# wangxuanx/Face-Diffusion-Model

Measured on AMD Instinct MI355X. Metric: animated frames/sec (1000-step DDPM, VOCASET FDM) at 1/2/4/8 MI355X, higher is better.
Workload: dtype bf16; 1 GPU; cfg2: vocaset FDM, 4 clips/GPU x 200 latent frames, 1000-step DDPM, random-init weights, synthetic audio-encoder features, Philox noise; global_batch=4, latent_frames=200, diffusion_steps=1000, parallelism=clip-shard x1

## Files before the change

face-diffusion-model_amd/csrc/fdm_hip.hip:

```cpp
#include <hip/hip_runtime.h>

#include <cstdarg>
#include <cstdio>
#include <functional>

#include "elementwise.hpp"
#include "window.hpp"
#include "slots.hpp"
#include "host.hpp"

namespace fdm {
thread_local std::string g_err;
int fail(int code, const char* fmt, ...) {
  char buf[512];
  va_list ap;
  va_start(ap, fmt);
  vsnprintf(buf, sizeof(buf), fmt, ap);
  va_end(ap);
  g_err = buf;
  return code;
}
}

namespace {
// ... 10 lines not shown
struct fdm_prog {
  std::vector<Op> ops;
  hipGraph_t graph = nullptr;
  hipGraphExec_t exec = nullptr;
};

namespace {

thread_local fdm_prog* g_rec = nullptr;

int submit(Op op, void* stream, const char* what) {
  if (g_rec) {
    g_rec->ops.push_back(std::move(op));
    return FDM_OK;
  }
  hipError_t e = op((hipStream_t)stream);
  if (e != hipSuccess) return hip_fail(e, what);
  return FDM_OK;
}

bool aligned16(const void* p) { return (((uintptr_t)p) & 15) == 0; }

}

extern "C" {

const char* fdm_last_error(void) { return g_err.c_str(); }
int fdm_version(void) { return 105; }

int fdm_abi_struct_size(const char* name) {
  if (!name) return fdm::fail(FDM_ERR_ARG, "abi_struct_size: null name");
  const std::string n(name);
  if (n == "fdm_sched_args") return (int)sizeof(fdm_sched_args);
  if (n == "fdm_gemm_args") return (int)sizeof(fdm_gemm_args);
  if (n == "fdm_attn_args") return (int)sizeof(fdm_attn_args);
  if (n == "fdm_ln_args") return (int)sizeof(fdm_ln_args);
  if (n == "fdm_model_desc") return (int)sizeof(fdm_model_desc);
  if (n == "fdm_sample_args") return (int)sizeof(fdm_sample_args);
  if (n == "fdm_vq_desc") return (int)sizeof(fdm_vq_desc);
  if (n == "fdm_slot_group_args") return (int)sizeof(fdm_slot_group_args);
  if (n == "fdm_slot_bank_args") return (int)sizeof(fdm_slot_bank_args);
  return fdm::fail(FDM_ERR_ARG, "abi_struct_size: unknown struct '%s'", name);
}

int fdm_device_ok(void) {
  int n = 0;
  if (hipGetDeviceCount(&n) != hipSuccess || n <= 0) return 0;
  hipDeviceProp_t prop;
  if (hipGetDeviceProperties(&prop, 0) != hipSuccess) return 0;
  return strncmp(prop.gcnArchName, "gfx950", 6) == 0 ? 1 : 0;
}

static bool gemm_act_heavy_host(int act) { return act == FDM_ACT_MISH || act == FDM_ACT_GELU_ERF || act == FDM_ACT_GELU_TANH; }

int fdm_op_gemm(const fdm_gemm_args* a, void* stream) {
  if (!a || !a->A || !a->W) return fail(FDM_ERR_ARG, "gemm: null operand");
  if (a->M <= 0 || a->N <= 0 || a->K <= 0) return fail(FDM_ERR_SHAPE, "gemm: M,N,K must be positive (%d,%d,%d)", a->M, a->N, a->K);
  if (!kind_ok(a->dtype)) return fail(FDM_ERR_ARG, "gemm: bad dtype %d", a->dtype);
  const bool split = kind(a->dtype).planes == 2;
  const int bk = kind(a->dtype).bk, epc = kind(a->dtype).epc;
  if (split && (a->a_lo_off <= 0 || a->w_lo_off <= 0 || a->a_lo_off % epc || a->w_lo_off % epc))
    return fail(FDM_ERR_ARG, "gemm: split operands need positive a_lo_off / w_lo_off (multiples of 8 elements)");
  if (split && a->out_t && a->out_t_lo_off <= 0) return fail(FDM_ERR_ARG, "gemm: split out_t needs out_t_lo_off");
  if (a->K % bk) return fail(FDM_ERR_SHAPE, "gemm: K=%d not a multiple of %d", a->K, bk);
  if (a->lda % epc || a->ldw % epc || !aligned16(a->A) || !aligned16(a->W)) return fail(FDM_ERR_ARG, "gemm: operands need 16-byte aligned rows");
  if (a->lda < 0 || a->ldw < 0 || a->lda > 0x7fffffffLL || a->ldw > 0x7fffffffLL) return fail(FDM_ERR_SHAPE, "gemm: lda / ldw are passed to the kernel as 32-bit element counts");
  if (a->a_batch_stride % epc || a->w_batch_stride % epc) return fail(FDM_ERR_ARG, "gemm: batch strides need 16-byte alignment");
  if (!a->out_f32 && !a->out_t && !a->out_vp && !a->out_kp) return fail(FDM_ERR_ARG, "gemm: no output");
  if (a->out_kp || a->out_vp) {
    const int hi = a->out_vp ? a->vp_col0 : a->N;
    if (a->kv_hd <= 0 || a->kv_hd % 16 || a->kv_L <= 0 || a->kv_Lpad < a->kv_L || a->kv_Lpad % 32 || a->M % a->kv_L)
      return fail(FDM_ERR_SHAPE, "gemm: bad packed K/V geometry (hd %d, L %d, Lpad %d)", a->kv_hd, a->kv_L, a->kv_Lpad);
    if (a->out_vp && (a->vp_col0 < 0 || a->vp_col0 % 4 || (a->N - a->vp_col0) % a->kv_hd)) return fail(FDM_ERR_SHAPE, "gemm: bad packed V column range");
    if (a->out_kp && (a->kp_col0 < 0 || a->kp_col0 % 4 || hi < a->kp_col0 || (hi - a->kp_col0) % a->kv_hd)) return fail(FDM_ERR_SHAPE, "gemm: bad packed K column range");
    if (!aligned16(a->out_kp) || !aligned16(a->out_vp)) return fail(FDM_ERR_ARG, "gemm: packed K/V buffers must be 16-byte aligned");
    if (a->dtype == FDM_F16X3 && (a->kv_lo_off <= 0 || a->kv_lo_off % 8)) return fail(FDM_ERR_ARG, "gemm: split packed K/V outputs need kv_lo_off");
  }
  if (a->bias && !aligned16(a->bias)) return fail(FDM_ERR_ARG, "gemm: bias must be 16-byte aligned");
  if (a->ln_stat_in && (a->ln_nparts <= 0 || a->ln_dim <= 0)) return fail(FDM_ERR_ARG, "gemm: ln_stat_in needs ln_nparts and ln_dim");
  if ((a->ln_colsum || a->rln_gamma) && !a->ln_stat_in) return fail(FDM_ERR_ARG, "gemm: LayerNorm folding needs ln_stat_in");
  if (a->rln_gamma && (!a->rln_beta || !a->resid)) return fail(FDM_ERR_ARG, "gemm: rln_gamma needs rln_beta and resid");
  if ((a->stat_out || a->ln_stat_in) && (a->batch > 1 || a->out_batch_stride)) return fail(FDM_ERR_ARG, "gemm: LayerNorm folding is not batched");
  if (a->tile < 0 || (a->tile & FDM_TILE_ID_MASK) > FDM_TILE_MAX) return fail(FDM_ERR_ARG, "gemm: unknown tile %d", a->tile);
  if (a->sched_fuse) {
    const fdm_sched_args& sc = a->sched;
    if (sc.mode != 0 && sc.mode != 1 && sc.mode != 3) return fail(FDM_ERR_ARG, "gemm: fused scheduler supports mode 0 (DDPM), 1 (DDIM) and 3 (table-driven)");
    if (!a->resid || !a->out_f32 || a->N % 64 || a->ldo_f32 != a->N || a->ldr != a->N || a->resid_row_mod || a->batch > 1 ||
        !aligned16(a->resid) || !aligned16(a->out_f32) || (a->out_t && (a->ldo_t != a->N || !aligned16(a->out_t))))
      return fail(FDM_ERR_SHAPE, "gemm: fused scheduler needs resid = x_t and out_f32 = x_{t-1} as dense [M, N] arrays, N %% 64 == 0");
    if (gemm_act_heavy_host(a->act) || a->stat_out || a->out_kp || a->out_vp || a->rln_gamma)
      return fail(FDM_ERR_ARG, "gemm: fused scheduler cannot be combined with Mish/GELU, stat_out, packed K/V or rln outputs");
    if (sc.mode == 0 && (!sc.c1 || !sc.c2 || !sc.sigma)) return fail(FDM_ERR_ARG, "gemm: fused DDPM needs c1, c2, sigma");
    if (sc.mode == 1 && (!sc.sra || !sc.srm1 || !sc.sqrt_an || !sc.c_n)) return fail(FDM_ERR_ARG, "gemm: fused DDIM needs sra, srm1, sqrt_an, c_n");
    if (sc.mode == 0 && !sc.noise && sc.n_per_clip <= 0) return fail(FDM_ERR_ARG, "gemm: fused DDPM with Philox noise needs n_per_clip");
    if (sc.mode == 3 && (!sc.lm_a || !sc.lm_b || !sc.lm_c || !sc.lm_s || !sc.x0_hist || !aligned16(sc.x0_hist)))
      return fail(FDM_ERR_ARG, "gemm: fused table-driven sampler needs lm_a, lm_b, lm_c, lm_s and a 16-byte aligned x0_hist [M, N]");
    if (sc.mode == 3 && !sc.noise && sc.n_per_clip <= 0) return fail(FDM_ERR_ARG, "gemm: fused table-driven sampler with Philox noise needs n_per_clip");
  }
  if (a->ksplit < 0 || a->ksplit > 4) return fail(FDM_ERR_ARG, "gemm: ksplit %d outside 0..4", a->ksplit);
  if (a->ksplit > 1) {
    const int tl = a->tile & FDM_TILE_ID_MASK;
    if (a->batch > 1 || a->out_batch_stride || a->act != FDM_ACT_NONE || !a->out_f32 || a->out_t || a->out_kp || a->out_vp || a->stat_out || a->ln_stat_in ||
        a->sched_fuse || a->resid_row_mod || (a->tile & FDM_TILE_GENERAL))
      return fail(FDM_ERR_ARG, "gemm: ksplit needs a plain launch (one batch, no activation, out_f32 as the only output, no folds)");
    if ((a->K / bk) % a->ksplit) return fail(FDM_ERR_SHAPE, "gemm: ksplit %d does not divide the %d k-tiles of K=%d", a->ksplit, a->K / bk, a->K);
    if (a->N % 64 || a->ldo_f32 % 4 || !aligned16(a->out_f32) || a->ksplit_stride % 4 || a->ksplit_stride < (long long)(a->M - 1) * a->ldo_f32 + a->N ||
        (a->resid && (a->ldr % 4 || !aligned16(a->resid))))
      return fail(FDM_ERR_SHAPE, "gemm: ksplit needs N %% 64 == 0, 16-byte aligned rows and ksplit_stride >= one output plane");
    if (tl != 0 && tl != FDM_TILE_64x64 && tl != FDM_TILE_64x64_S2 && tl != FDM_TILE_32x64_S3)
      return fail(FDM_ERR_ARG, "gemm: ksplit runs on the 64-column tiles (FDM_TILE_64x64, FDM_TILE_64x64_S2, FDM_TILE_32x64_S3), not tile %d", tl);
  }
  if (a->batch2 < 0) return fail(FDM_ERR_ARG, "gemm: negative batch2");
  if (a->batch2 >= 1) {
    const int tl = a->tile & FDM_TILE_ID_MASK;
    if (a->ksplit > 1 || a->out_kp || a->out_vp || a->stat_out || a->ln_stat_in || a->sched_fuse || a->resid_row_mod || a->incr_counter)
      return fail(FDM_ERR_ARG, "gemm: batch2 cannot be combined with ksplit, packed K/V, LayerNorm folds, the fused scheduler or resid_row_mod");
    if (a->a_batch_stride2 % epc) return fail(FDM_ERR_ARG, "gemm: a_batch_stride2 needs 16-byte alignment");
    if (tl != 0 && tl != FDM_TILE_64x64 && tl != FDM_TILE_64x64_S2 && tl != FDM_TILE_128x64)
      return fail(FDM_ERR_ARG, "gemm: batch2 runs on the 64-column tiles (FDM_TILE_64x64, FDM_TILE_64x64_S2, FDM_TILE_128x64), not tile %d", tl);
    if (a->batch < 1) return fail(FDM_ERR_ARG, "gemm: batch2 needs batch >= 1 (the group count of the second batch level)");
  }
  fdm_gemm_args c = *a;
  return submit([c](hipStream_t s) { return fdm::gemm_launch(c, s); }, stream, "gemm");
}

int fdm_gemm_heuristic_tile(const fdm_gemm_args* a) {
  if (!a) return fail(FDM_ERR_ARG, "gemm_heuristic_tile: null argument");
  return fdm::gemm_heuristic_tile_of(*a);
}

int fdm_op_attention(const fdm_attn_args* a, void* stream) {
  if (!a || !a->Q || !a->Kp || !a->Vp || !a->O) return fail(FDM_ERR_ARG, "attention: null operand");
  if (a->hd != 64 && a->hd != 128 && a->hd != 256) return fail(FDM_ERR_SHAPE, "attention: head_dim %d unsupported (64, 128, 256)", a->hd);
  if (a->B <= 0 || a->H <= 0 || a->L <= 0) return fail(FDM_ERR_SHAPE, "attention: B,H,L must be positive");
  if (a->Lpad < a->L || a->Lpad % 32) return fail(FDM_ERR_SHAPE, "attention: Lpad=%d must be a multiple of 32 >= L", a->Lpad);
  if (!kind_ok(a->dtype)) return fail(FDM_ERR_ARG, "attention: bad dtype %d (FDM_F32, FDM_BF16, FDM_F16X3, FDM_F16)", a->dtype);
  if (a->o_split && (a->dtype != FDM_F32 || a->o_split != FDM_F16X3 || a->o_lo_off <= 0))
    return fail(FDM_ERR_ARG, "attention: o_split needs dtype FDM_F32, a split kind and o_lo_off");
  if (a->dtype == FDM_F16X3 && (a->q_lo_off <= 0 || a->kv_lo_off <= 0 || a->o_lo_off <= 0 || a->q_lo_off % 8 || a->kv_lo_off % 8 || a->o_lo_off % 4))
    return fail(FDM_ERR_ARG, "attention: split operands need q_lo_off, kv_lo_off and o_lo_off");
  if (a->q_lo_off > 0x7fffffffLL || a->kv_lo_off > 0x7fffffffLL || a->ldq > 0x7fffffffLL)
    return fail(FDM_ERR_SHAPE, "attention: q_lo_off, kv_lo_off and ldq are passed to the kernel as 32-bit element counts");
  const int epc = kind(a->dtype).epc;
  if (a->ldq % epc || a->ldo % 4 || !aligned16(a->Q) || !aligned16(a->Kp) || !aligned16(a->Vp) || !aligned16(a->O))
    return fail(FDM_ERR_ARG, "attention: operands need 16-byte aligned rows");
  if (a->slopes && a->period <= 0) return fail(FDM_ERR_ARG, "attention: period must be positive");
  if (a->lens && (a->causal || (a->hd != 64 && a->hd != 128)))
    return fail(FDM_ERR_ARG, "attention: per-clip lengths need causal = 0 and head_dim 64 or 128");
  fdm_attn_args c = *a;
  return submit([c](hipStream_t s) { return fdm::attn_launch(c, s); }, stream, "attention");
}

int fdm_op_pack_kv(const void* K, long long ldk, const void* V, long long ldv, void* Kp, void* Vp,
                   int B, int H, int L, int Lpad, int hd, int dtype, void* stream) {
  if (!K || !V || !Kp || !Vp) return fail(FDM_ERR_ARG, "pack_kv: null operand");
  if (B <= 0 || H <= 0 || L <= 0 || Lpad < L || Lpad % 32 || hd <= 0 || hd % 16) return fail(FDM_ERR_SHAPE, "pack_kv: bad geometry");
  if (dtype != FDM_F32 && dtype != FDM_BF16) return fail(FDM_ERR_ARG, "pack_kv: bad dtype %d", dtype);
  return submit([=](hipStream_t s) {
    return dtype == FDM_BF16 ? fdm::pack_kv_launch_bf16(K, ldk, V, ldv, Kp, Vp, B, H, L, Lpad, hd, s)
                             : fdm::pack_kv_launch_f32(K, ldk, V, ldv, Kp, Vp, B, H, L, Lpad, hd, s);
  }, stream, "pack_kv");
}

int fdm_op_layernorm(const fdm_ln_args* a, void* stream) {
  if (!a || !a->x || !a->gamma || !a->beta) return fail(FDM_ERR_ARG, "layernorm: null operand");
  if (a->d != 256 && a->d != 512 && a->d != 768 && a->d != 1024) return fail(FDM_ERR_SHAPE, "layernorm: d=%d unsupported (256, 512, 768, 1024)", a->d);
  if (a->M <= 0) return fail(FDM_ERR_SHAPE, "layernorm: M must be positive");
  if (!a->y_f32 && !a->y_t) return fail(FDM_ERR_ARG, "layernorm: no output");
  if (!kind_ok(a->dtype)) return fail(FDM_ERR_ARG, "layernorm: bad dtype %d", a->dtype);
  if (a->y_t && a->dtype == FDM_F16X3 && (a->y_t_lo_off <= 0 || a->y_t_lo_off % 4)) return fail(FDM_ERR_ARG, "layernorm: split y_t needs y_t_lo_off");
  if (a->add_mat_group < 0 || a->add_mat_wrap < 0 ||
      (a->add_mat_group > 0 && (a->add_mat_L <= 0 || a->add_mat_group % a->add_mat_L || (a->add_mat_wrap > 0 && a->add_mat_wrap % a->add_mat_group))))
    return fail(FDM_ERR_SHAPE, "layernorm: shared add_mat needs add_mat_L | add_mat_group | add_mat_wrap (got %d, %d, %d)", a->add_mat_L, a->add_mat_group, a->add_mat_wrap);
  if (a->x_planes < 0 || a->x_planes > 4 || (a->x_planes > 1 && (a->x_plane_stride < (long long)a->M * a->d || a->x_plane_stride % 4)))
    return fail(FDM_ERR_ARG, "layernorm: x_planes %d (0..4) needs x_plane_stride >= M * d, a multiple of 4", a->x_planes);
  if (a->clip_step && (a->clip_rows <= 0 || a->clip_step_stride <= 0 || a->clip_wrap < 0 || (a->clip_wrap > 0 && a->clip_wrap % a->clip_rows)))
    return fail(FDM_ERR_SHAPE, "layernorm: clip_step needs clip_rows > 0, clip_step_stride > 0 and clip_rows | clip_wrap (got %d, %d, %d)", a->clip_rows, a->clip_step_stride, a->clip_wrap);
  if (a->clip_step && a->act != FDM_ACT_NONE && a->act != FDM_ACT_RELU) return fail(FDM_ERR_ARG, "layernorm: clip_step runs with FDM_ACT_NONE / FDM_ACT_RELU only");
  fdm_ln_args c = *a;
  return submit([c](hipStream_t s) {
    switch (c.dtype) {
      case FDM_BF16: return fdm::ln_launch_t<fdm::bf16>(c, s);
      case FDM_F16X3: return fdm::ln_launch_t<fdm::f16x3_t>(c, s);
      case FDM_F16: return fdm::ln_launch_t<fdm::f16>(c, s);
      default: return fdm::ln_launch_t<float>(c, s);
    }
  }, stream, "layernorm");
}

int fdm_op_sched_step(const fdm_sched_args* a, void* stream) {
  if (!a || !a->x0 || !a->x_out) return fail(FDM_ERR_ARG, "sched: null operand");
  if (a->n <= 0 || a->n % 4) return fail(FDM_ERR_SHAPE, "sched: n=%lld must be a positive multiple of 4", a->n);
  if (a->mode == 0 && (!a->x || !a->c1 || !a->c2 || !a->sigma)) return fail(FDM_ERR_ARG, "sched: DDPM tables missing");
  if (a->mode == 1 && (!a->x || !a->sra || !a->srm1 || !a->sqrt_an || !a->c_n)) return fail(FDM_ERR_ARG, "sched: DDIM tables missing");
  if (a->mode == 3 && (!a->x || !a->lm_a || !a->lm_b || !a->lm_c || !a->lm_s || !a->x0_hist)) return fail(FDM_ERR_ARG, "sched: table-driven sampler needs lm_a, lm_b, lm_c, lm_s, x0_hist");
  if (a->mode < 0 || a->mode > 3) return fail(FDM_ERR_ARG, "sched: bad mode %d", a->mode);
  if (a->mode == 3 && !a->noise && (a->n_per_clip <= 0 || a->n_per_clip % 4)) return fail(FDM_ERR_SHAPE, "sched: n_per_clip must be a positive multiple of 4");
  if (a->mode == 0 && !a->noise && (a->n_per_clip <= 0 || a->n_per_clip % 4)) return fail(FDM_ERR_SHAPE, "sched: n_per_clip must be a positive multiple of 4");
  if (a->x_out_t && !kind_ok(a->out_dtype)) return fail(FDM_ERR_ARG, "sched: bad out_dtype %d", a->out_dtype);
  if (a->x_out_t && a->out_dtype == FDM_F16X3 && (a->x_out_t_lo_off <= 0 || a->x_out_t_lo_off % 4)) return fail(FDM_ERR_ARG, "sched: split x_out_t needs x_out_t_lo_off");
  fdm_sched_args c = *a;
  return submit([c](hipStream_t s) { return fdm::sched_launch(c, s); }, stream, "sched");
}

int fdm_op_slot_sched(const fdm_sched_args* a, const int* state, const unsigned long long* keys, int n_slots, void* stream) {
  if (!a || !a->x0 || !a->x || !a->x_out || !state || !keys) return fail(FDM_ERR_ARG, "slot_sched: null operand");
  if (a->noise) return fail(FDM_ERR_ARG, "slot_sched: injected noise is not supported (Philox keyed per slot)");
  if (a->mode != 0 && a->mode != 1 && a->mode != 3) return fail(FDM_ERR_ARG, "slot_sched: mode %d (0 DDPM, 1 DDIM, 3 table-driven)", a->mode);
  if (n_slots < 1 || a->n_per_clip <= 0 || a->n_per_clip % 4 || a->n != (long long)n_slots * a->n_per_clip)
    return fail(FDM_ERR_SHAPE, "slot_sched: n=%lld must be n_slots=%d x n_per_clip=%lld (a multiple of 4)", a->n, n_slots, a->n_per_clip);
  if (a->mode == 0 && (!a->c1 || !a->c2 || !a->sigma)) return fail(FDM_ERR_ARG, "slot_sched: DDPM tables missing");
// ... 531 lines not shown
```

face-diffusion-model_amd/csrc/gemm.hpp:

```cpp
#pragma once
#include <cstdlib>
#include <cstring>

#include "common.hpp"
#include "sched.hpp"
#include "../../include/fdm_hip.h"

namespace fdm {

template <int BM, int BN> constexpr int gemm_ln_scratch_bytes() { return BM * 2 * 4; }
template <typename T, int BM, int BN> constexpr int gemm_epi_ring_bytes() {
  using KK = typename Opnd<T>::KV;
  return BM * BN * (int)sizeof(typename Opnd<KK>::E) * Opnd<KK>::NP + BM * 2 * (BN / 16) * 4;
}

template <int BM>
__device__ __forceinline__ void gemm_load_rowstats(const fdm_gemm_args& p, int m0, float* rowstat) {
  if (!p.ln_stat_in) return;
  const int t = threadIdx.x;
  if (t < BM) {
    const int m = min(m0 + t, p.M - 1);
    float s = 0.f, q = 0.f;
    typedef __attribute__((ext_vector_type(2))) float f32x2;
    for (int i0 = 0; i0 < p.ln_nparts; i0 += 16) {
      f32x2 v[16];
#pragma unroll
      for (int i = 0; i < 16; ++i) {
        const int ii = min(i0 + i, p.ln_nparts - 1);
        v[i] = *(const f32x2*)(p.ln_stat_in + ((size_t)ii * p.M + m) * 2);
      }
#pragma unroll
      for (int i = 0; i < 16; ++i)
        if (i0 + i < p.ln_nparts) { s += v[i][0]; q += v[i][1]; }
    }
    const float inv = 1.f / (float)p.ln_dim;
    const float mu = s * inv;
    const float var = fmaxf(q * inv - mu * mu, 0.f);
    rowstat[2 * t] = mu;
    rowstat[2 * t + 1] = 1.f / sqrtf(var + p.ln_eps);
  }
  asm volatile("s_waitcnt lgkmcnt(0)" ::: "memory");
}

template <int MI, int NI> struct EpiPre { f32x4 csv[NI], bv[NI], gmv[NI], btv[NI], rv[MI][NI]; SchedCoef sc; };

template <typename T, int BM, int BN, int WM, int WN, int SCHED = 0>
__device__ __forceinline__ void gemm_epi_preload(const fdm_gemm_args& p, int m0, int n0, int z, int wm, int wn, int g, int r16,
                                                 bool ln_capable, EpiPre<BM / WM / 16, BN / WN / 16>& e) {
  constexpr int MI = BM / WM / 16, NI = BN / WN / 16;
  if constexpr (SCHED != 0) e.sc = sched_coef_load<SCHED == 2>(p.sched);
  const int M = p.M, N = p.N;
  const bool use_ln = ln_capable && p.ln_stat_in;
  const float* bias = p.bias ? p.bias + (size_t)z * p.bias_batch_stride : nullptr;
  const size_t ocol = (size_t)z * p.out_batch_stride;
  const bool vec_r = p.resid && (p.ldr % 4 == 0) && (((uintptr_t)(p.resid + ocol)) % 16 == 0);
  const bool pre_cs = use_ln && p.ln_colsum, pre_rln = use_ln && p.rln_gamma && p.resid;
#pragma unroll
  for (int ni = 0; ni < NI; ++ni) {
    const int n = n0 + wn * (BN / WN) + ni * 16 + 4 * g;
    const bool full = (n + 3 < N);
    const f32x4 zero = f32x4{0.f, 0.f, 0.f, 0.f};
    e.csv[ni] = (pre_cs && full) ? *(const f32x4*)(p.ln_colsum + n) : zero;
    e.bv[ni] = (bias && full) ? *(const f32x4*)(bias + n) : zero;
    e.gmv[ni] = (pre_rln && full) ? *(const f32x4*)(p.rln_gamma + n) : zero;
    e.btv[ni] = (pre_rln && full) ? *(const f32x4*)(p.rln_beta + n) : zero;
#pragma unroll
    for (int mi = 0; mi < MI; ++mi) {
      const int m = m0 + wm * (BM / WM) + mi * 16 + r16;
      const size_t rrow = p.resid_row_mod > 0 ? (size_t)(min(m, M - 1) % p.resid_row_mod) : (size_t)min(m, M - 1);
      e.rv[mi][ni] = (p.resid && vec_r && full && m < M) ? *(const f32x4*)(p.resid + ocol + rrow * p.ldr + n) : zero;
    }
  }
}

template <bool HEAVY, typename T> __device__ __forceinline__ float gemm_act(float v, int act) {
  if constexpr (!HEAVY) {
    return act == ACT_RELU ? fmaxf(v, 0.f) : (act == ACT_LEAKY02 ? (v > 0.f ? v : 0.2f * v) : v);
  } else if constexpr (is_fast16<T>::value) {
    if (act == ACT_MISH) {
      const float sp = v > 20.f ? v : __logf(1.f + __expf(v));
      return v * (1.f - 2.f / (1.f + __expf(2.f * sp)));
    }
    if (act == ACT_GELU_TANH) {
      const float c = 0.7978845608028654f * (v + 0.044715f * v * v * v);
      return v * (0.5f * (2.f - 2.f / (1.f + __expf(2.f * c))));
    }
    return act_apply_t<T>(v, act);
  } else {
    return act_apply(v, act);
  }
}
__host__ __device__ inline bool gemm_act_is_heavy(int act) { return act == ACT_MISH || act == ACT_GELU_ERF || act == ACT_GELU_TANH; }

constexpr int GEMM_LEAN = 1, GEMM_KV = 2, GEMM_FOLD = 4, GEMM_KSPLIT = 8, GEMM_B2 = 16, GEMM_LM = 32;
template <int MODE> struct KSliceArgs;
template <> struct KSliceArgs<0> {
  const fdm_gemm_args& a;
  __device__ __forceinline__ KSliceArgs(const fdm_gemm_args& p, int, int) : a(p) {}
};
template <> struct KSliceArgs<1> {
  fdm_gemm_args a;
  __device__ __forceinline__ KSliceArgs(const fdm_gemm_args& p, int slice, int) : a(p) {
    a.out_f32 = p.out_f32 + (size_t)slice * p.ksplit_stride;
    if (slice > 0) { a.bias = nullptr; a.resid = nullptr; }
  }
};
template <> struct KSliceArgs<2> {
  fdm_gemm_args a;
  __device__ __forceinline__ KSliceArgs(const fdm_gemm_args& p, int c, int out_t_elem_bytes) : a(p) {
    const size_t off = (size_t)c * p.out_batch_stride2;
    if (p.out_f32) a.out_f32 = p.out_f32 + off;
    if (p.resid) a.resid = p.resid + off;
    if (p.out_t) a.out_t = (char*)p.out_t + off * out_t_elem_bytes;
  }
};
template <typename T, int BM, int BN, int WM = 2, int WN = 2, bool HEAVY = true, bool SCHED = false, int SPEC = 0>
__device__ __forceinline__ void gemm_epilogue(const fdm_gemm_args& p, f32x4 (&acc)[BM / WM / 16][BN / WN / 16],
                                              const EpiPre<BM / WM / 16, BN / WN / 16>& e, int m0, int n0, int z,
                                              int wm, int wn, int g, int r16, float* rowstat = nullptr, char* tile_lds = nullptr) {
  constexpr int MI = BM / WM / 16, NI = BN / WN / 16;
  constexpr bool LEAN = (SPEC & GEMM_LEAN) != 0;
  constexpr bool KVC = !LEAN || (SPEC & GEMM_KV), FOLDC = !LEAN || (SPEC & GEMM_FOLD);
  using E = typename Opnd<T>::E;
  using KK = typename Opnd<T>::KV;
  using KV = typename Opnd<KK>::E;
  constexpr int KNP = Opnd<KK>::NP;
  const int M = p.M, N = p.N;
  constexpr int EPC_T = 16 / (int)sizeof(KV);
  const bool vt_tile = KVC && tile_lds && p.out_vp && n0 >= p.vp_col0 && n0 + BN <= N && (p.kv_L % EPC_T == 0);
  KV* tl = (KV*)tile_lds;
  float* comb = tile_lds ? (float*)(tile_lds + BM * BN * (int)sizeof(KV) * KNP) : nullptr;
  const bool use_ln = FOLDC && rowstat && p.ln_stat_in;
  const bool do_stat = FOLDC && rowstat && comb && p.stat_out;
  if (vt_tile || do_stat) __syncthreads();
  const float* bias = p.bias ? p.bias + (size_t)z * p.bias_batch_stride : nullptr;
  const size_t ocol = (size_t)z * p.out_batch_stride;
  const bool vec_f32 = p.out_f32 && (p.ldo_f32 % 4 == 0) && (((uintptr_t)(p.out_f32 + ocol)) % 16 == 0);
  const bool vec_t = p.out_t && (p.ldo_t % 4 == 0) && (((uintptr_t)((E*)p.out_t + ocol)) % (4 * sizeof(E)) == 0) &&
                     (Opnd<T>::NP == 1 || p.out_t_lo_off % 4 == 0);
  const bool vec_r = p.resid && (p.ldr % 4 == 0) && (((uintptr_t)(p.resid + ocol)) % 16 == 0);
  const int kv_H = p.out_vp ? (N - p.vp_col0) / p.kv_hd : 0;
  const size_t kv_blk = (size_t)p.kv_Lpad * p.kv_hd;
  const int kcol_lo = p.out_kp ? p.kp_col0 : N, kcol_hi = p.out_kp ? (p.out_vp ? p.vp_col0 : N) : N;
  const bool pre_cs = use_ln && p.ln_colsum, pre_rln = use_ln && p.rln_gamma && p.resid;
  const f32x4 (&csv)[NI] = e.csv; const f32x4 (&bv)[NI] = e.bv; const f32x4 (&gmv)[NI] = e.gmv; const f32x4 (&btv)[NI] = e.btv;
  const f32x4 (&rv)[MI][NI] = e.rv;
  const int kv_mode = (!KVC || (!p.out_kp && !p.out_vp)) ? 0
                    : (n0 + BN <= (p.out_kp ? kcol_lo : p.vp_col0)) ? 0
                    : (p.out_kp && n0 >= kcol_lo && n0 + BN <= kcol_hi) ? 1
                    : vt_tile ? 2
                    : (p.out_vp && n0 >= p.vp_col0 && n0 + BN <= N) ? 3 : -1;
  const bool lean = LEAN || (kv_mode >= 0 && n0 + BN <= N && (vec_f32 || !p.out_f32) && (vec_t || !p.out_t) && (vec_r || !p.resid) &&
                            (p.kv_hd % 16 == 0 || kv_mode != 1));
  if (lean) {
    const int ncol = n0 + wn * (BN / WN) + 4 * g;
    const int KH = (kv_mode == 1) ? (kcol_hi - kcol_lo) / p.kv_hd : 1;
#pragma unroll
    for (int mi = 0; mi < MI; ++mi) {
      const int lrow = wm * (BM / WM) + mi * 16 + r16;
      const int m = m0 + lrow;
      if (m >= M) continue;
      const float mu = use_ln ? rowstat[2 * lrow] : 0.f, rs = use_ln ? rowstat[2 * lrow + 1] : 1.f;
      float* o32 = p.out_f32 ? p.out_f32 + ocol + (size_t)m * p.ldo_f32 + ncol : nullptr;
      E* ot = p.out_t ? (E*)p.out_t + ocol + (size_t)m * p.ldo_t + ncol : nullptr;
      KV* okp = nullptr;
      int kv_l = 0;
      if (kv_mode == 1) {
        const int kv_b = m / p.kv_L;
        kv_l = m - kv_b * p.kv_L;
        okp = (KV*)p.out_kp + (size_t)kv_b * KH * kv_blk;
      } else if (kv_mode == 3) {
        const int kv_b = m / p.kv_L;
        kv_l = m - kv_b * p.kv_L;
        okp = (KV*)p.out_vp + (size_t)kv_b * kv_H * kv_blk;
      }
#pragma unroll
      for (int ni = 0; ni < NI; ++ni) {
        f32x4 v = acc[mi][ni];
        if (pre_cs) v = (v - mu * csv[ni]) * rs;
        if (bias) v += bv[ni];
        if (p.act != ACT_NONE) {
#pragma unroll
          for (int j = 0; j < 4; ++j) v[j] = gemm_act<HEAVY, T>(v[j], p.act);
        }
        if constexpr (SCHED) {
          v = sched_update4<(SPEC & GEMM_LM) != 0>(p.sched, e.sc, v, rv[mi][ni], (long long)m * N + (ncol + ni * 16));
        } else {
          if (p.resid) v += pre_rln ? (rv[mi][ni] - mu) * rs * gmv[ni] + btv[ni] : rv[mi][ni];
        }
        if (do_stat) {
          const float fs = rows_sum((v[0] + v[1]) + (v[2] + v[3]));
          const float fq = rows_sum((v[0] * v[0] + v[1] * v[1]) + (v[2] * v[2] + v[3] * v[3]));
          if (g == 0) { float* cb = comb + ((size_t)(wn * NI + ni) * BM + lrow) * 2; cb[0] = fs; cb[1] = fq; }
        }
        if (kv_mode == 2) {
          const int nl = wn * (BN / WN) + ni * 16 + 4 * g;
#pragma unroll
          for (int j = 0; j < 4; ++j) store_opnd1<KK>(tl + (nl + j) * BM + lrow, BM * BN, v[j]);
          continue;
        }
        if (kv_mode == 1) {
          const int cc = ncol + ni * 16 - kcol_lo;
          const int h = cc / p.kv_hd, e2 = cc - h * p.kv_hd;
          store_opnd4<KK>(okp + (size_t)h * kv_blk + kp_offset<KV>(kv_l, e2, p.kv_hd), p.kv_lo_off, v);
          continue;
        }
        if (kv_mode == 3) {
          const int cc = ncol + ni * 16 - p.vp_col0;
          const int h = cc / p.kv_hd, e2 = cc - h * p.kv_hd;
#pragma unroll
// ... 81 lines not shown
          if (n + j >= N) break;
          const int cc = n + j - p.vp_col0;
          const int h = cc / p.kv_hd, e = cc - h * p.kv_hd;
          store_opnd1<KK>((KV*)p.out_vp + (size_t)(kv_b * kv_H + h) * kv_blk + vp_offset<KV>(kv_l, e, p.kv_hd), p.kv_lo_off, v[j]);
        }
        continue;
      }
      if (p.out_f32) {
        float* op = p.out_f32 + ocol + (size_t)m * p.ldo_f32 + n;
        if (full && vec_f32) {
          *(f32x4*)op = v;
        } else {
          for (int j = 0; j < 4; ++j)
            if (n + j < N) op[j] = v[j];
        }
      }
      if (p.out_t) {
        E* op = (E*)p.out_t + ocol + (size_t)m * p.ldo_t + n;
        if (full && vec_t) {
          store_opnd4<T>(op, p.out_t_lo_off, v);
        } else {
          for (int j = 0; j < 4; ++j)
            if (n + j < N) store_opnd1<T>(op + j, p.out_t_lo_off, v[j]);
        }
      }
    }
  }
  }
  if (vt_tile) {
    __syncthreads();
    constexpr int CPR = BM / EPC_T;
    for (int c = threadIdx.x; c < BN * CPR; c += WM * WN * 64) {
      const int nl = c / CPR, ml = (c % CPR) * EPC_T;
      const int m = m0 + ml;
      if (m >= M) continue;
      const int b = m / p.kv_L, l = m - b * p.kv_L;
      const int cc = n0 + nl - p.vp_col0;
      const int h = cc / p.kv_hd, e = cc - h * p.kv_hd;
#pragma unroll
      for (int pl = 0; pl < KNP; ++pl)
        *(u32x4*)((KV*)p.out_vp + (size_t)pl * p.kv_lo_off + (size_t)(b * kv_H + h) * kv_blk + vp_offset<KV>(l, e, p.kv_hd)) =
            *(const u32x4*)(tl + pl * BM * BN + nl * BM + ml);
    }
  }
  if (do_stat) {
    __syncthreads();
    const int t = threadIdx.x;
    if (t < BM && m0 + t < M) {
#pragma unroll
      for (int gq = 0; gq < BN / 64; ++gq) {
        if (n0 + gq * 64 >= N) break;
        float s = 0.f, q = 0.f;
#pragma unroll
        for (int f = 0; f < 4; ++f) { s += comb[((size_t)(gq * 4 + f) * BM + t) * 2]; q += comb[((size_t)(gq * 4 + f) * BM + t) * 2 + 1]; }
        float* so = p.stat_out + ((size_t)(n0 / 64 + gq) * M + (m0 + t)) * 2;
        so[0] = s; so[1] = q;
      }
    }
  }
}

#ifndef FDM_LW_VARIANT
#define FDM_LW_VARIANT 0
#endif
typedef __attribute__((address_space(1))) const void* gptr_t;
typedef __attribute__((address_space(3))) void* lptr_t;

template <int N> __device__ __forceinline__ void wait_vmcnt() { asm volatile("s_waitcnt vmcnt(%0)" ::"n"(N) : "memory"); }

template <typename T, int BM, int BN, int WM, int WN, int NST, int KCH = 8, bool HEAVY = false, bool SCHED = false, int SPEC = 0, int LW = 0>
__global__ __launch_bounds__(64 * (WM * WN + LW)) void gemm_glds_kernel(const void* pA, const void* pW, long long p_a_lo_off, long long p_w_lo_off,
                                                                        int pM, int pN, int pK, int p_lda, int p_ldw, const fdm_gemm_args p) {
  using E = typename Opnd<T>::E;
  constexpr int NP = Opnd<T>::NP;
  constexpr int NW = WM * WN;
  constexpr int ROWB = KCH * 16;
  constexpr int RPI = 1024 / ROWB;
  constexpr int MI = BM / WM / 16, NI = BN / WN / 16;
  constexpr int NA = BM / RPI, NWP = BN / RPI;
  constexpr int IW = LW > 0 ? LW : NW;
  constexpr bool UNEVEN = NA % IW != 0;
  static_assert(NWP % IW == 0 && BM % RPI == 0 && MI >= 1 && NI >= 1, "tile does not fit the wave grid");
  constexpr int A_IPW = (NA + IW - 1) / IW, W_IPW = NWP / IW;
  constexpr int P = NP * (A_IPW + W_IPW), P_LO = NP * (A_IPW - 1 + W_IPW);
  constexpr int STAGE = NP * (BM + BN) * ROWB;
  static_assert(NST * STAGE >= gemm_epi_ring_bytes<T, BM, BN>(), "epilogue staging does not fit in the ring");
  constexpr bool EARLY_READS = NP * (KCH / 4) * (MI + NI) <= 12;
  extern __shared__ __attribute__((aligned(16))) char smem[];
#ifdef FDM_GEMM_STAMPS
  const unsigned long long t_first = wall_clock64();
#endif
  float* rowstat = (float*)(smem + NST * STAGE);

  const int tid = threadIdx.x, lane = tid & 63;
#ifdef FDM_GEMM_STAMPS
  unsigned long long* stamps = (!p.incr_counter && p.incr_table) ? (unsigned long long*)p.incr_table + (size_t)(blockIdx.y * gridDim.x + blockIdx.x) * 8 : nullptr;
  if (stamps && tid == 0) { stamps[0] = wall_clock64(); stamps[5] = t_first; }
#endif
  const int wave_id = __builtin_amdgcn_readfirstlane(tid >> 6);
  const bool loader = LW > 0 && wave_id >= NW;
  const int wave = LW > 0 ? (loader ? wave_id - NW : 0) : wave_id;
  const int wm = wave_id / WN, wn = wave_id % WN;
  const int g = lane >> 4, r16 = lane & 15;
  constexpr bool KSP = (SPEC & GEMM_KSPLIT) != 0, B2 = (SPEC & GEMM_B2) != 0;
  int z = KSP ? 0 : blockIdx.z;
  int by = blockIdx.y, bx = blockIdx.x, c2 = 0;
  if constexpr (B2) {
    const int nx = gridDim.x, ny = gridDim.y, G = p.batch > 0 ? p.batch : 1, C = p.batch2;
    const int id = (blockIdx.z * ny + blockIdx.y) * nx + blockIdx.x;
    int g_, r;
    if (G % 8 == 0) {
      const int per_g = ny * nx * C, slot = id >> 3;
      const int gl = slot / per_g;
      g_ = (id & 7) * (G / 8) + gl; r = slot - gl * per_g;
    } else {
      const int per_g = ny * nx * C;
      g_ = id / per_g; r = id - g_ * per_g;
    }
    z = g_; c2 = r / (ny * nx);
    const int r2 = r - c2 * ny * nx;
    by = r2 / nx; bx = r2 - by * nx;
  }
  const int m0 = by * BM, n0 = bx * BN;
  const int M = pM, N = pN;
  constexpr int EPC = 16 / (int)sizeof(E);
  int nk = pK / (KCH * EPC);
  const E* A = (const E*)pA;
  const E* W = (const E*)pW;
  if (z) {
    A += (size_t)z * p.a_batch_stride;
    W += (size_t)z * p.w_batch_stride;
  }
  if constexpr (KSP) {
    nk /= p.ksplit;
    A += (size_t)blockIdx.z * nk * (KCH * EPC);
    W += (size_t)blockIdx.z * nk * (KCH * EPC);
  }
  if constexpr (B2) A += (size_t)c2 * p.a_batch_stride2;
  const KSliceArgs<KSP ? 1 : (B2 ? 2 : 0)> ksa(p, KSP ? (int)blockIdx.z : c2, (int)sizeof(E));
  const fdm_gemm_args& pe = ksa.a;
  const size_t a_lo = (size_t)p_a_lo_off * sizeof(E), w_lo = (size_t)p_w_lo_off * sizeof(E);

  const int lrow = lane / KCH, slot = lane % KCH;
  const char* a_src[A_IPW];
  const char* w_src[W_IPW];
#pragma unroll
  for (int i = 0; i < A_IPW; ++i) {
    const int piece = UNEVEN ? min(i * IW + wave, NA - 1) : wave * A_IPW + i;
    const int row = RPI * piece + lrow;
    a_src[i] = (const char*)(A + (size_t)min(m0 + row, M - 1) * p_lda) + ((slot ^ (row % KCH)) << 4);
  }
#pragma unroll
  for (int i = 0; i < W_IPW; ++i) {
    const int row = RPI * (wave * W_IPW + i) + lrow;
    w_src[i] = (const char*)(W + (size_t)min(n0 + row, N - 1) * p_ldw) + ((slot ^ (row % KCH)) << 4);
  }
  auto issue = [&](int kt) {
    char* sb = smem + (kt % NST) * STAGE;
    const size_t off = (size_t)kt * ROWB;
#pragma unroll
    for (int pl = 0; pl < NP; ++pl) {
#pragma unroll
      for (int i = 0; i < A_IPW; ++i) {
        if constexpr (UNEVEN) {
          if (i * IW + wave < NA)
            __builtin_amdgcn_global_load_lds((gptr_t)(a_src[i] + off + pl * a_lo), (lptr_t)(sb + pl * BM * ROWB + (i * IW + wave) * 1024), 16, 0, 0);
        } else {
          __builtin_amdgcn_global_load_lds((gptr_t)(a_src[i] + off + pl * a_lo), (lptr_t)(sb + pl * BM * ROWB + (wave * A_IPW + i) * 1024), 16, 0, 0);
        }
      }
#pragma unroll
      for (int i = 0; i < W_IPW; ++i)
        __builtin_amdgcn_global_load_lds((gptr_t)(w_src[i] + off + pl * w_lo), (lptr_t)(sb + (NP * BM + pl * BN) * ROWB + (wave * W_IPW + i) * 1024), 16, 0, 0);
    }
  };

  f32x4 acc[MI][NI];
  f32x4 accl[NP == 2 ? MI : 1][NP == 2 ? NI : 1];
#pragma unroll
  for (int mi = 0; mi < MI; ++mi)
#pragma unroll
    for (int ni = 0; ni < NI; ++ni) {
      acc[mi][ni] = f32x4{0.f, 0.f, 0.f, 0.f};
      if constexpr (NP == 2) accl[mi][ni] = f32x4{0.f, 0.f, 0.f, 0.f};
    }

  if (LW == 0 || loader) {
#pragma unroll
    for (int t = 0; t < NST - 1; ++t)
      if (t < nk) issue(t);
  }
  if (p.incr_counter && tid == 0 && blockIdx.x == 0 && blockIdx.y == 0 && blockIdx.z == 0) {
    const int nv = *p.incr_counter + 1;
    *p.incr_counter = nv;
    if (p.incr_table) p.incr_counter[1] = p.incr_table[nv];
  }
  if constexpr (LW > 0) {
    if (loader) {
      for (int kt = 0; kt < nk; ++kt) {
        if (kt + NST - 2 < nk) {
          if (!UNEVEN || wave < NA % IW) wait_vmcnt<(NST - 2) * P>();
          else wait_vmcnt<(NST - 2) * P_LO>();
        } else {
          wait_vmcnt<0>();
        }
        __builtin_amdgcn_s_barrier();
        if constexpr (!(FDM_LW_VARIANT & 4)) { if (kt + NST - 1 < nk) issue(kt + NST - 1); }
      }
      return;
    }
  }
  EpiPre<MI, NI> epre;
  constexpr bool FOLDC = !(SPEC & GEMM_LEAN) || (SPEC & GEMM_FOLD);
  gemm_epi_preload<T, BM, BN, WM, WN, (SCHED ? ((SPEC & GEMM_LM) ? 2 : 1) : 0)>(pe, m0, n0, z, wm, wn, g, r16, FOLDC, epre);
  if constexpr (FOLDC) gemm_load_rowstats<BM>(p, m0, rowstat);

  auto frag_a = [&](const char* base, int pl, int s, int mi) {
    const int row = wm * (BM / WM) + mi * 16 + r16;
    return *(const u32x4*)(base + (pl * BM + row) * ROWB + (((4 * s + g) ^ (row % KCH)) << 4));
  };
  auto frag_w = [&](const char* base, int pl, int s, int ni) {
    const int row = wn * (BN / WN) + ni * 16 + r16;
    return *(const u32x4*)(base + (NP * BM + pl * BN + row) * ROWB + (((4 * s + g) ^ (row % KCH)) << 4));
  };
  auto mma = [&](int mi, int ni, const u32x4 (&wf)[NP], const u32x4 (&af)[NP]) {
    if constexpr (NP == 1) {
      Mma<T>::run(acc[mi][ni], wf[0], af[0]);
    } else {
      mma16<E>(acc[mi][ni], wf[0], af[0]);
      mma16<E>(accl[mi][ni], wf[0], af[1]);
      mma16<E>(accl[mi][ni], wf[1], af[0]);
    }
  };

  for (int kt = 0; kt < nk; ++kt) {
    if constexpr (LW == 0) {
      if (kt + NST - 2 < nk) {
        if (!UNEVEN || wave < NA % IW) wait_vmcnt<(NST - 2) * P>();
        else wait_vmcnt<(NST - 2) * P_LO>();
      } else {
        wait_vmcnt<0>();
      }
    }
    __builtin_amdgcn_s_barrier();
#ifdef FDM_GEMM_STAMPS
    if (stamps && tid == 0 && kt == 0) stamps[1] = wall_clock64();
#endif
    const char* base = smem + (kt % NST) * STAGE;
    if constexpr (EARLY_READS) {
      u32x4 af[KCH / 4][MI][NP], wf[KCH / 4][NI][NP];
#pragma unroll
      for (int s = 0; s < KCH / 4; ++s)
#pragma unroll
        for (int pl = 0; pl < NP; ++pl) {
#pragma unroll
          for (int mi = 0; mi < MI; ++mi) af[s][mi][pl] = (FDM_LW_VARIANT & 2) ? u32x4{(unsigned)kt, 1u, 2u, 3u} : frag_a(base, pl, s, mi);
#pragma unroll
          for (int ni = 0; ni < NI; ++ni) wf[s][ni][pl] = (FDM_LW_VARIANT & 2) ? u32x4{(unsigned)kt, 5u, 6u, 7u} : frag_w(base, pl, s, ni);
        }
      if (LW == 0 && kt + NST - 1 < nk) issue(kt + NST - 1);
#pragma unroll
      for (int s = 0; s < KCH / 4; ++s)
#pragma unroll
        for (int mi = 0; mi < MI; ++mi)
#pragma unroll
          for (int ni = 0; ni < NI; ++ni) {
            if constexpr (FDM_LW_VARIANT & 1) { asm volatile("" ::"v"(wf[s][ni][0]), "v"(af[s][mi][0])); }
            else mma(mi, ni, wf[s][ni], af[s][mi]);
          }
    } else {
      if (LW == 0 && kt + NST - 1 < nk) issue(kt + NST - 1);
#pragma unroll
      for (int s = 0; s < KCH / 4; ++s) {
        u32x4 af[MI][NP], wf[NI][NP];
#pragma unroll
        for (int pl = 0; pl < NP; ++pl) {
#pragma unroll
          for (int mi = 0; mi < MI; ++mi) af[mi][pl] = (FDM_LW_VARIANT & 2) ? u32x4{(unsigned)kt, 1u, 2u, 3u} : frag_a(base, pl, s, mi);
#pragma unroll
          for (int ni = 0; ni < NI; ++ni) wf[ni][pl] = (FDM_LW_VARIANT & 2) ? u32x4{(unsigned)kt, 5u, 6u, 7u} : frag_w(base, pl, s, ni);
        }
#pragma unroll
        for (int mi = 0; mi < MI; ++mi)
#pragma unroll
          for (int ni = 0; ni < NI; ++ni) {
            if constexpr (FDM_LW_VARIANT & 1) { asm volatile("" ::"v"(wf[ni][0]), "v"(af[mi][0])); }
            else mma(mi, ni, wf[ni], af[mi]);
          }
      }
    }
  }
  if constexpr (NP == 2) {
    constexpr float inv = 1.f / Opnd<T>::SCALE;
#pragma unroll
    for (int mi = 0; mi < MI; ++mi)
#pragma unroll
      for (int ni = 0; ni < NI; ++ni) acc[mi][ni] += accl[mi][ni] * inv;
  }
#ifdef FDM_GEMM_STAMPS
  if (stamps && tid == 0) stamps[2] = wall_clock64();
#endif
  if constexpr (LW > 0) wait_vmcnt<0>();
#ifndef FDM_GEMM_STAMPS
  gemm_epilogue<T, BM, BN, WM, WN, HEAVY, SCHED, SPEC>(pe, acc, epre, m0, n0, z, wm, wn, g, r16, rowstat, smem);
#else
  const int passes = (stamps && p.sched.advance == 2 && !SCHED) ? 2 : 1;
#pragma clang loop unroll(disable)
  for (int pass = 0; pass < passes; ++pass) {
    gemm_epilogue<T, BM, BN, WM, WN, HEAVY, SCHED, SPEC>(pe, acc, epre, m0, n0, z, wm, wn, g, r16, rowstat, smem);
    if (stamps && tid == 0) stamps[pass == 0 ? 3 : 6] = wall_clock64();
    asm volatile("s_waitcnt vmcnt(0)" ::: "memory");
    __syncthreads();
    if (stamps && tid == 0) stamps[pass == 0 ? 4 : 7] = wall_clock64();
  }
#endif
}

#ifndef FDM_PP_PRIO
#define FDM_PP_PRIO 1
#endif
#ifndef FDM_PP_VARIANT
#define FDM_PP_VARIANT 0
#endif
template <typename T, int BM, int BN, int WM, int WN, int NST, bool HEAVY = false, bool SCHED = false, int SPEC = 0, int KCH = 8>
__global__ __launch_bounds__(512) void gemm_pp_kernel(const fdm_gemm_args p) {
  using E = typename Opnd<T>::E;
  static_assert(WM * WN == 8, "ping-pong loop: two groups of four waves");
  constexpr int NP = Opnd<T>::NP;
  static_assert(KCH == 8 || KCH == 4, "LDS rows of 128 or 64 bytes");
  constexpr int NW = 8, ROWB = KCH * 16, RPI = 1024 / ROWB, KS = KCH / 4;
  constexpr int MI = BM / WM / 16, NI = BN / WN / 16;
  constexpr int A_IPW = BM / RPI / NW, W_IPW = BN / RPI / NW;
  static_assert(A_IPW >= 1 && W_IPW >= 1 && MI >= 1 && NI >= 1, "tile too small for the wave grid");
  constexpr int P = NP * (A_IPW + W_IPW);
  constexpr int D = NST - 1;
  constexpr int STAGE = NP * (BM + BN) * ROWB;
  constexpr bool EPI_RING = !(SPEC & GEMM_LEAN) || (SPEC & (GEMM_KV | GEMM_FOLD));
  static_assert(NST >= 2 && (!EPI_RING || NST * STAGE >= gemm_epi_ring_bytes<T, BM, BN>()), "epilogue staging does not fit in the ring");
  extern __shared__ __attribute__((aligned(16))) char smem[];
  float* rowstat = (float*)(smem + NST * STAGE);
#ifdef FDM_PP_PHASES
  const unsigned long long t_entry = wall_clock64();
#endif

  const int tid = threadIdx.x, lane = tid & 63;
  if (p.incr_counter && tid == 0 && blockIdx.x == 0 && blockIdx.y == 0 && blockIdx.z == 0) {
    const int nv = *p.incr_counter + 1;
    *p.incr_counter = nv;
    if (p.incr_table) p.incr_counter[1] = p.incr_table[nv];
  }
  const int wave = __builtin_amdgcn_readfirstlane(tid >> 6);
  const int grp = wave >> 2;
  const int wm = wave / WN, wn = wave % WN;
  const int g = lane >> 4, r16 = lane & 15;
  const int z = blockIdx.z;
  const int gx = gridDim.x, gy = gridDim.y, nwg = gx * gy;
  int bid = blockIdx.y * gx + blockIdx.x;
  {
    const int q = nwg / 8, r = nwg % 8, xcd = bid % 8, idx = bid / 8;
    bid = (xcd < r ? xcd * (q + 1) : r * (q + 1) + (xcd - r) * q) + idx;
  }
  const int m0 = (bid / gx) * BM, n0 = (bid % gx) * BN;
  const int M = p.M, N = p.N;
  const E* A = (const E*)p.A + (size_t)z * p.a_batch_stride;
  const E* W = (const E*)p.W + (size_t)z * p.w_batch_stride;
  const size_t a_lo = (size_t)p.a_lo_off * sizeof(E), w_lo = (size_t)p.w_lo_off * sizeof(E);

  auto swz = [](int row) { return KCH == 8 ? (row & 7) : ((0x78 >> (2 * ((row >> 2) & 3))) & 3); };
  const int lrow = lane / KCH, slot = lane % KCH;
  const char* a_src[A_IPW];
  const char* w_src[W_IPW];
#pragma unroll
  for (int i = 0; i < A_IPW; ++i) {
    const int row = RPI * (wave * A_IPW + i) + lrow;
    a_src[i] = (const char*)(A + (size_t)min(m0 + row, M - 1) * p.lda) + ((slot ^ swz(row)) << 4);
  }
#pragma unroll
  for (int i = 0; i < W_IPW; ++i) {
    const int row = RPI * (wave * W_IPW + i) + lrow;
    w_src[i] = (const char*)(W + (size_t)min(n0 + row, N - 1) * p.ldw) + ((slot ^ swz(row)) << 4);
  }
  auto issue = [&](int kt) {
    char* sb = smem + (kt % NST) * STAGE;
    const size_t off = (size_t)kt * ROWB;
#pragma unroll
    for (int pl = 0; pl < NP; ++pl) {
#pragma unroll
      for (int i = 0; i < A_IPW; ++i)
        __builtin_amdgcn_global_load_lds((gptr_t)(a_src[i] + off + pl * a_lo), (lptr_t)(sb + pl * BM * ROWB + (wave * A_IPW + i) * 1024), 16, 0, 0);
#pragma unroll
      for (int i = 0; i < W_IPW; ++i)
        __builtin_amdgcn_global_load_lds((gptr_t)(w_src[i] + off + pl * w_lo), (lptr_t)(sb + (NP * BM + pl * BN) * ROWB + (wave * W_IPW + i) * 1024), 16, 0, 0);
// ... 74 lines not shown
  for (int kt = 0; kt < nk; ++kt) {
    PP_STAMP(0);
    if constexpr (FDM_PP_PRIO == 2) __builtin_amdgcn_s_setprio(1);
    if constexpr (!(FDM_PP_VARIANT & 2)) load_frags(kt);
    __builtin_amdgcn_sched_barrier(0);
    if constexpr (!(FDM_PP_VARIANT & 4)) { if (kt + D < nk) issue(kt + D); }
    if (grp) {
      if (kt + D < nk) wait_vmcnt<(D - 1) * P>(); else wait_vmcnt<0>();
    }
    __builtin_amdgcn_sched_barrier(0);
    if constexpr (FDM_PP_PRIO == 2) __builtin_amdgcn_s_setprio(0);
    PP_STAMP(1);
    asm volatile("s_waitcnt lgkmcnt(0)" ::: "memory");
    __builtin_amdgcn_s_barrier();
    PP_STAMP(2);
    __builtin_amdgcn_sched_barrier(0);
    if constexpr (FDM_PP_PRIO == 1) __builtin_amdgcn_s_setprio(1);
    if constexpr (!(FDM_PP_VARIANT & 1)) {
      compute();
    } else if constexpr (!(FDM_PP_VARIANT & 2)) {
#pragma unroll
      for (int s = 0; s < KS; ++s) {
#pragma unroll
        for (int mi = 0; mi < MI; ++mi) asm volatile("" ::"v"(af[s][mi][0]));
#pragma unroll
        for (int ni = 0; ni < NI; ++ni) asm volatile("" ::"v"(wf[s][ni][0]));
      }
    }
    if constexpr (FDM_PP_PRIO == 1) __builtin_amdgcn_s_setprio(0);
    if (!grp) {
      if (kt + D < nk) wait_vmcnt<(D - 1) * P>(); else wait_vmcnt<0>();
    }
    __builtin_amdgcn_sched_barrier(0);
    PP_STAMP(3);
    __builtin_amdgcn_s_barrier();
  }
  if (!grp) __builtin_amdgcn_s_barrier();
#ifdef FDM_PP_PHASES
  if (phases) phases[2] = wall_clock64();
#endif
  if constexpr (NP == 2) {
    constexpr float inv = 1.f / Opnd<T>::SCALE;
#pragma unroll
    for (int mi = 0; mi < MI; ++mi)
#pragma unroll
      for (int ni = 0; ni < NI; ++ni) acc[mi][ni] += accl[mi][ni] * inv;
  }
  if constexpr (MI > 4 && !EPI_RING) {
#pragma unroll
    for (int hh = 0; hh < 2; ++hh) {
      f32x4 (&acch)[MI / 2][NI] = *reinterpret_cast<f32x4 (*)[MI / 2][NI]>(&acc[hh * (MI / 2)]);
      const int m0h = m0 + wm * (BM / WM) - wm * (BM / 2 / WM) + hh * (BM / 2 / WM);
      EpiPre<MI / 2, NI> epre;
      gemm_epi_preload<T, BM / 2, BN, WM, WN, (SCHED ? ((SPEC & GEMM_LM) ? 2 : 1) : 0)>(p, m0h, n0, z, wm, wn, g, r16, false, epre);
      gemm_epilogue<T, BM / 2, BN, WM, WN, HEAVY, SCHED, SPEC>(p, acch, epre, m0h, n0, z, wm, wn, g, r16, nullptr, nullptr);
    }
  } else {
    EpiPre<MI, NI> epre;
    gemm_epi_preload<T, BM, BN, WM, WN, (SCHED ? ((SPEC & GEMM_LM) ? 2 : 1) : 0)>(p, m0, n0, z, wm, wn, g, r16, FOLDC, epre);
    gemm_epilogue<T, BM, BN, WM, WN, HEAVY, SCHED, SPEC>(p, acc, epre, m0, n0, z, wm, wn, g, r16, rowstat, smem);
  }
#ifdef FDM_PP_PHASES
  asm volatile("s_waitcnt vmcnt(0)" ::: "memory");
  __syncthreads();
  if (phases) phases[3] = wall_clock64();
#endif
}

template <typename T, int BM, int BN, int WM, int WN, int NST, bool HEAVY, bool SCHED = false, int SPEC = 0, int KCH = 8>
static hipError_t gemm_pp_launch_h(const fdm_gemm_args& a, hipStream_t s) {
  dim3 grid((a.N + BN - 1) / BN, (a.M + BM - 1) / BM, a.batch > 0 ? a.batch : 1);
  constexpr int lds = NST * Opnd<T>::NP * (BM + BN) * KCH * 16 + gemm_ln_scratch_bytes<BM, BN>();
  static_assert(lds <= 160 * 1024, "ring does not fit the CU's LDS");
  static bool once = [] {
    return hipFuncSetAttribute((const void*)gemm_pp_kernel<T, BM, BN, WM, WN, NST, HEAVY, SCHED, SPEC, KCH>, hipFuncAttributeMaxDynamicSharedMemorySize, lds) == hipSuccess;
  }();
  (void)once;
  hipLaunchKernelGGL((gemm_pp_kernel<T, BM, BN, WM, WN, NST, HEAVY, SCHED, SPEC, KCH>), grid, dim3(512), lds, s, a);
  return hipGetLastError();
}

template <typename T, int BM, int BN, int WM, int WN, int NST, int KCH, bool HEAVY, bool SCHED = false, int SPEC = 0, int LW = 0>
static hipError_t gemm_glds_launch_h(const fdm_gemm_args& a, hipStream_t s) {
  dim3 grid((a.N + BN - 1) / BN, (a.M + BM - 1) / BM, (SPEC & GEMM_KSPLIT) ? a.ksplit : (a.batch > 0 ? a.batch : 1) * ((SPEC & GEMM_B2) ? a.batch2 : 1));
  constexpr int lds = NST * Opnd<T>::NP * (BM + BN) * KCH * 16 + gemm_ln_scratch_bytes<BM, BN>();
  static_assert(lds <= 160 * 1024, "ring does not fit the CU's LDS");
  static bool once = [] {
    return hipFuncSetAttribute((const void*)gemm_glds_kernel<T, BM, BN, WM, WN, NST, KCH, HEAVY, SCHED, SPEC, LW>, hipFuncAttributeMaxDynamicSharedMemorySize, lds) == hipSuccess;
  }();
  (void)once;
  hipLaunchKernelGGL((gemm_glds_kernel<T, BM, BN, WM, WN, NST, KCH, HEAVY, SCHED, SPEC, LW>), grid, dim3(64 * (WM * WN + LW)), lds, s,
                     a.A, a.W, (long long)a.a_lo_off, (long long)a.w_lo_off, a.M, a.N, a.K, (int)a.lda, (int)a.ldw, a);
  return hipGetLastError();
}
static bool gemm_lockstep_env() {
  static bool v = [] { const char* e = getenv("FDM_GEMM_LOCKSTEP"); return e && atoi(e) != 0; }();
  return v;
}
template <typename T, int BM, int BN>
static bool gemm_all_tiles_lean(const fdm_gemm_args& a) {
  using E = typename Opnd<T>::E;
  auto al = [](const void* p, size_t n) { return ((uintptr_t)p % n) == 0; };
  if (a.N % BN || a.out_batch_stride % 4 || a.resid_row_mod) return false;
  if (a.out_f32 && (a.ldo_f32 % 4 || !al(a.out_f32, 16))) return false;
  if (a.out_t && (a.ldo_t % 4 || !al(a.out_t, 4 * sizeof(E)) || (Opnd<T>::NP == 2 && a.out_t_lo_off % 4))) return false;
  if (a.resid && (a.ldr % 4 || !al(a.resid, 16))) return false;
  if (a.out_kp || a.out_vp) {
    const int kcol_lo = a.out_kp ? a.kp_col0 : a.N, kcol_hi = a.out_kp ? (a.out_vp ? a.vp_col0 : a.N) : a.N;
    if (a.kv_hd % 16) return false;
    if (a.out_kp && (kcol_lo % BN || kcol_hi % BN)) return false;
    if (a.out_vp && a.vp_col0 % BN) return false;
    if (!a.out_kp && a.out_vp) return false;
  }
  return true;
}
template <typename T, int BM, int BN, int WM, int WN, int NST, int KCH, int LW>
static hipError_t gemm_glds_launch_lw(const fdm_gemm_args& a, hipStream_t s) {
  const bool no_lean = (a.tile & FDM_TILE_GENERAL) != 0;
  if (a.ksplit > 1) {
    if constexpr (BN == 64 && (BM == 64 || BM == 32)) {
      if (!gemm_all_tiles_lean<T, BM, BN>(a)) return hipErrorInvalidValue;
      return gemm_glds_launch_h<T, BM, BN, WM, WN, NST, KCH, false, false, GEMM_LEAN | GEMM_KSPLIT, LW>(a, s);
    } else {
      return hipErrorInvalidValue;
    }
  }
  if (a.batch2 >= 1) {
    if constexpr (BN == 64 && (BM == 64 || BM == 128)) {
      if (!no_lean && gemm_all_tiles_lean<T, BM, BN>(a) && a.out_batch_stride2 % 4 == 0)
        return gemm_glds_launch_h<T, BM, BN, WM, WN, NST, KCH, true, false, GEMM_LEAN | GEMM_B2, LW>(a, s);
      return gemm_glds_launch_h<T, BM, BN, WM, WN, NST, KCH, true, false, GEMM_B2, LW>(a, s);
    } else {
      return hipErrorInvalidValue;
    }
  }
  if (gemm_act_is_heavy(a.act)) {
    if (!no_lean && !a.out_kp && !a.out_vp && !a.stat_out && !a.ln_stat_in && gemm_all_tiles_lean<T, BM, BN>(a))
      return gemm_glds_launch_h<T, BM, BN, WM, WN, NST, KCH, true, false, GEMM_LEAN, LW>(a, s);
    return gemm_glds_launch_h<T, BM, BN, WM, WN, NST, KCH, true, false, 0, LW>(a, s);
  }
  if (!no_lean && gemm_all_tiles_lean<T, BM, BN>(a)) {
    const bool kv = a.out_kp || a.out_vp, fold = a.stat_out || a.ln_stat_in;
    if (kv && fold) return gemm_glds_launch_h<T, BM, BN, WM, WN, NST, KCH, false, false, GEMM_LEAN | GEMM_KV | GEMM_FOLD, LW>(a, s);
    if (kv) return gemm_glds_launch_h<T, BM, BN, WM, WN, NST, KCH, false, false, GEMM_LEAN | GEMM_KV, LW>(a, s);
    if (fold) return gemm_glds_launch_h<T, BM, BN, WM, WN, NST, KCH, false, false, GEMM_LEAN | GEMM_FOLD, LW>(a, s);
    return gemm_glds_launch_h<T, BM, BN, WM, WN, NST, KCH, false, false, GEMM_LEAN, LW>(a, s);
  }
  return gemm_glds_launch_h<T, BM, BN, WM, WN, NST, KCH, false, false, 0, LW>(a, s);
}

template <typename T, int BM, int BN, int WM, int WN, int NST, int LW_ = 0, int KCH = 8>
static hipError_t gemm_glds_launch_t(const fdm_gemm_args& a, hipStream_t s) {
  if constexpr (LW_ > 0 && !std::is_same<T, float>::value) {
    if (!(a.tile & FDM_TILE_LOCKSTEP) && !gemm_lockstep_env()) return gemm_glds_launch_lw<T, BM, BN, WM, WN, NST, KCH, LW_>(a, s);
  }
  return gemm_glds_launch_lw<T, BM, BN, WM, WN, NST, KCH, 0>(a, s);
}

template <typename T, int BM, int BN, int WM, int WN, int NST>
static hipError_t gemm_pp_launch_t(const fdm_gemm_args& a, hipStream_t s) {
  const bool no_lean = (a.tile & FDM_TILE_GENERAL) != 0;
  if (gemm_act_is_heavy(a.act)) {
    if (!no_lean && !a.out_kp && !a.out_vp && !a.stat_out && !a.ln_stat_in && gemm_all_tiles_lean<T, BM, BN>(a))
      return gemm_pp_launch_h<T, BM, BN, WM, WN, NST, true, false, GEMM_LEAN>(a, s);
    return gemm_pp_launch_h<T, BM, BN, WM, WN, NST, true>(a, s);
  }
  if (!no_lean && gemm_all_tiles_lean<T, BM, BN>(a)) {
    const bool kv = a.out_kp || a.out_vp, fold = a.stat_out || a.ln_stat_in;
    if (kv && fold) return gemm_pp_launch_h<T, BM, BN, WM, WN, NST, false, false, GEMM_LEAN | GEMM_KV | GEMM_FOLD>(a, s);
    if (kv) return gemm_pp_launch_h<T, BM, BN, WM, WN, NST, false, false, GEMM_LEAN | GEMM_KV>(a, s);
    if (fold) return gemm_pp_launch_h<T, BM, BN, WM, WN, NST, false, false, GEMM_LEAN | GEMM_FOLD>(a, s);
    return gemm_pp_launch_h<T, BM, BN, WM, WN, NST, false, false, GEMM_LEAN>(a, s);
  }
  return gemm_pp_launch_h<T, BM, BN, WM, WN, NST, false>(a, s);
}

static int gemm_tile_override() {
  static int v = [] { const char* e = getenv("FDM_GEMM_TILE"); return e ? atoi(e) : 0; }();
  return v;
}
static bool gemm_one_round(long long tiles) { return tiles > 192 && tiles <= 256; }
static bool gemm_one_round_80(const fdm_gemm_args& a) {
  const long long t80 = (long long)((a.M + 79) / 80) * ((a.N + 127) / 128) * (a.batch > 0 ? a.batch : 1);
  return t80 > 224 && t80 <= 256 && (a.M % 80 == 0 || a.M % 80 > 40);
}

static bool gemm_one_round_64x128(const fdm_gemm_args& a) {
  const long long t = (long long)((a.M + 63) / 64) * ((a.N + 127) / 128) * (a.batch > 0 ? a.batch : 1);
  return gemm_one_round(t) && a.N >= 2048 && a.N % 128 == 0;
}

static int gemm_heuristic_tile(const fdm_gemm_args& a, int elem_bytes, bool split) {
  if (a.batch2 >= 1) {
    const long long t128b = (long long)((a.M + 127) / 128) * ((a.N + 63) / 64) * (a.batch > 0 ? a.batch : 1) * a.batch2;
    return t128b >= 192 ? FDM_TILE_128x64 : FDM_TILE_64x64;
  }
  const long long batch = a.batch > 0 ? a.batch : 1;
  const long long t128 = (long long)((a.M + 127) / 128) * ((a.N + 127) / 128) * batch;
  const long long t128x64 = (long long)((a.M + 127) / 128) * ((a.N + 63) / 64) * batch;
  const long long t64 = (long long)((a.M + 63) / 64) * ((a.N + 63) / 64) * batch;
  const long long t64x128 = (long long)((a.M + 63) / 64) * ((a.N + 127) / 128) * batch;
  const bool narrow_one_round = elem_bytes == 2 && a.N <= 512 && a.N % 128 == 0 && t64 > 256 && t64x128 <= 256;
  const bool wide_128x64 = elem_bytes == 2 && a.M <= 1024 && a.N >= 2048 && t128x64 >= 160 && t128x64 <= 256;
  if (!split) {
    constexpr long long thr128 = 512, thr128x64 = 700;
    const long long t256 = (long long)((a.M + 255) / 256) * ((a.N + 127) / 128) * batch;
    const bool pp_ok = elem_bytes == 2 && a.N % 128 == 0 && a.K >= 1024;
    if (pp_ok && a.M >= 6000 && a.N <= 2048 && t256 >= 150) return FDM_TILE_256x128_PP;
    if (elem_bytes == 2 && a.M > 1024 && t128 >= thr128 && gemm_one_round(t256)) return FDM_TILE_256x128_PP;
    if (t128 >= thr128) {
      const long long tail = t128 % 256;
      if (elem_bytes == 2 && t128 < 1024 && tail > 0 && tail < 128) return FDM_TILE_128x64;
      return FDM_TILE_128x128;
    }
    if (gemm_one_round_80(a)) return FDM_TILE_80x128;
    if (elem_bytes == 2 && gemm_one_round_64x128(a)) return FDM_TILE_64x128;
    if (wide_128x64) return FDM_TILE_128x64;
    if (narrow_one_round && a.M > 1024) return FDM_TILE_64x128;
    if (elem_bytes == 2 && t64 <= 128 && a.N <= 1536) return FDM_TILE_32x64_S3;
    if (elem_bytes == 2 && a.M > 1024 && (t64 > 512 || a.K >= 1024)) {
      if (gemm_one_round(t128)) return FDM_TILE_128x128;
      if (gemm_one_round(t256)) return FDM_TILE_256x128_PP;
      if (t128x64 > 128) return FDM_TILE_128x64;
    }
    if (t128x64 >= thr128x64) return FDM_TILE_128x64;
    return FDM_TILE_64x64;
  }
  if (t128 >= 512) return FDM_TILE_128x128;
  if (gemm_one_round_80(a)) return FDM_TILE_80x128;
  if (gemm_one_round_64x128(a)) return FDM_TILE_64x128;
  if (wide_128x64) return FDM_TILE_128x64;
  if (a.M > 1024) {
    if (gemm_one_round(t128)) return FDM_TILE_128x128;
    if (narrow_one_round) return FDM_TILE_64x128;
    if (t128x64 > 128 && t128x64 <= 256) return FDM_TILE_128x64;
    struct { int id, bm, bn; } cand[] = {{FDM_TILE_64x64, 64, 64}, {FDM_TILE_128x64, 128, 64}, {FDM_TILE_64x128, 64, 128}, {FDM_TILE_80x128, 80, 128}, {FDM_TILE_128x128, 128, 128}};
    int best = FDM_TILE_64x64; long long best_rows = -1;
    for (auto& c : cand) {
      if (a.N % c.bn) continue;
      const long long tiles = (long long)((a.M + c.bm - 1) / c.bm) * (a.N / c.bn) * batch;
      const long long rows = ((tiles + 255) / 256) * (c.bm + c.bn);
      if (best_rows < 0 || rows < best_rows) { best = c.id; best_rows = rows; }
    }
    return best;
  } else {
    if (t64 <= 128) return FDM_TILE_32x64_S3;
    if (t64 > 256 && t64x128 <= 256 && a.N % 128 == 0) return FDM_TILE_64x128;
    if (t64 > 256 && t64 <= 512 && a.N >= 2048) return FDM_TILE_64x64_S2;
  }
  if (t128x64 >= 700) return FDM_TILE_128x64;
  return FDM_TILE_64x64;
}

static bool gemm_sched_fuse_heuristic_pp(const fdm_gemm_args& a, int elem_bytes) {
  fdm_gemm_args b = a;
  b.sched_fuse = 0;
  return gemm_heuristic_tile(b, elem_bytes, false) == FDM_TILE_256x128_PP;
}

template <typename T, int LM = 0>
static hipError_t gemm_sched_fuse_launch(const fdm_gemm_args& a, hipStream_t s) {
  if constexpr (LM == 0) {
    if (a.sched.mode == 3) return gemm_sched_fuse_launch<T, GEMM_LM>(a, s);
  }
  if constexpr (!std::is_same<T, float>::value) {
    if (!(a.tile & FDM_TILE_LOCKSTEP) && !gemm_lockstep_env())
      return a.ln_stat_in ? gemm_glds_launch_h<T, 64, 64, 2, 4, 4, 8, false, true, GEMM_LEAN | GEMM_FOLD | LM, 4>(a, s)
                          : gemm_glds_launch_h<T, 64, 64, 2, 4, 4, 8, false, true, GEMM_LEAN | LM, 4>(a, s);
  }
  return a.ln_stat_in ? gemm_glds_launch_h<T, 64, 64, 2, 4, 4, 8, false, true, GEMM_LEAN | GEMM_FOLD | LM>(a, s)
                      : gemm_glds_launch_h<T, 64, 64, 2, 4, 4, 8, false, true, GEMM_LEAN | LM>(a, s);
}

static int gemm_ksplit_heuristic_tile(const fdm_gemm_args& a) { return a.M <= 256 ? FDM_TILE_32x64_S3 : FDM_TILE_64x64; }
template <typename T>
static hipError_t gemm_dispatch_ksplit(const fdm_gemm_args& a, int tile_id, hipStream_t s) {
  switch (tile_id > 0 ? tile_id : gemm_ksplit_heuristic_tile(a)) {
    case FDM_TILE_64x64_S2: return gemm_glds_launch_t<T, 64, 64, 2, 4, 2, 4>(a, s);
    case FDM_TILE_32x64_S3: return gemm_glds_launch_t<T, 32, 64, 2, 2, 3, 2>(a, s);
    default: return gemm_glds_launch_t<T, 64, 64, 2, 4, 4, 4>(a, s);
  }
}

template <typename T>
static hipError_t gemm_dispatch(const fdm_gemm_args& a, hipStream_t s) {
  if (a.sched_fuse) {
    const int tile_id = a.tile & FDM_TILE_ID_MASK;
    const bool pp = tile_id == FDM_TILE_256x128_PP || (tile_id == 0 && gemm_tile_override() == 0 && gemm_sched_fuse_heuristic_pp(a, (int)sizeof(typename Opnd<T>::E)));
    if (pp && !a.ln_stat_in && a.N % 128 == 0)
      return a.sched.mode == 3 ? gemm_pp_launch_h<T, 256, 128, 4, 2, 3, false, true, GEMM_LEAN | GEMM_LM>(a, s)
                               : gemm_pp_launch_h<T, 256, 128, 4, 2, 3, false, true, GEMM_LEAN>(a, s);
    return gemm_sched_fuse_launch<T>(a, s);
  }
  const int tile_id = a.tile & FDM_TILE_ID_MASK;
  if (a.ksplit > 1) return gemm_dispatch_ksplit<T>(a, tile_id, s);
  const int want = tile_id > 0 ? tile_id : (a.batch2 >= 1 ? 0 : gemm_tile_override());
  switch (want > 0 ? want : gemm_heuristic_tile(a, (int)sizeof(typename Opnd<T>::E), false)) {
    case FDM_TILE_128x64_S3:
    case FDM_TILE_128x64: {
      const long long wgs = (long long)((a.M + 127) / 128) * ((a.N + 63) / 64) * (a.batch > 0 ? a.batch : 1) * (a.batch2 > 0 ? a.batch2 : 1);
      return wgs <= 256 ? gemm_glds_launch_t<T, 128, 64, 4, 2, 4, 4>(a, s) : gemm_glds_launch_t<T, 128, 64, 4, 2, 3, 4>(a, s);
    }
    case FDM_TILE_96x128:
    case FDM_TILE_128x128: return gemm_glds_launch_t<T, 128, 128, 2, 4, 3, 4>(a, s);
    case FDM_TILE_64x64_S2: return gemm_glds_launch_t<T, 64, 64, 2, 4, 2, 4>(a, s);
    case FDM_TILE_32x64_S3: return gemm_glds_launch_t<T, 32, 64, 2, 2, 3, 2>(a, s);
    case FDM_TILE_256x128:
    case FDM_TILE_256x128_PP: return gemm_pp_launch_t<T, 256, 128, 4, 2, 3>(a, s);
    case FDM_TILE_80x128: return gemm_glds_launch_t<T, 80, 128, 1, 8, 4, 4>(a, s);
    case FDM_TILE_64x128: return gemm_glds_launch_t<T, 64, 128, 2, 4, 4, 4>(a, s);
    default: return gemm_glds_launch_t<T, 64, 64, 2, 4, 4, 4>(a, s);
  }
}

template <typename T>
static hipError_t gemm_dispatch_split(const fdm_gemm_args& a, hipStream_t s) {
  if (a.sched_fuse)
    return gemm_sched_fuse_launch<T>(a, s);
  const int tile_id = a.tile & FDM_TILE_ID_MASK;
  if (a.ksplit > 1) return gemm_dispatch_ksplit<T>(a, tile_id, s);
  const int want = tile_id > 0 ? tile_id : (a.batch2 >= 1 ? 0 : gemm_tile_override());
  switch (want > 0 ? want : gemm_heuristic_tile(a, 2, true)) {
    case FDM_TILE_64x64_S2: return gemm_glds_launch_t<T, 64, 64, 2, 4, 2, 4>(a, s);
    case FDM_TILE_32x64_S3: return gemm_glds_launch_t<T, 32, 64, 2, 2, 3, 2>(a, s);
    case FDM_TILE_128x64:
    case FDM_TILE_128x64_S3: return gemm_glds_launch_t<T, 128, 64, 4, 2, 3, 4>(a, s);
    case FDM_TILE_128x128:
    case FDM_TILE_96x128:
    case FDM_TILE_256x128:
    case FDM_TILE_256x128_PP: return gemm_glds_launch_t<T, 128, 128, 2, 4, 2, 4>(a, s);
    case FDM_TILE_80x128: return gemm_glds_launch_t<T, 80, 128, 1, 8, 3, 4>(a, s);
    case FDM_TILE_64x128: return gemm_glds_launch_t<T, 64, 128, 2, 4, 3, 4>(a, s);
    default: return gemm_glds_launch_t<T, 64, 64, 2, 4, 4, 4>(a, s);
  }
}

}
```

face-diffusion-model_amd/csrc/gemm_bf16.hip:

```cpp
#include "gemm.hpp"
#include "kernels.hpp"
namespace fdm { hipError_t gemm_launch_bf16(const fdm_gemm_args& a, hipStream_t s) { return gemm_dispatch<bf16>(a, s); } }
namespace fdm {
int gemm_heuristic_tile_of(const fdm_gemm_args& a) {
  if (a.ksplit > 1) return gemm_ksplit_heuristic_tile(a);
  if (a.sched_fuse) {
    const bool pp = a.dtype != FDM_F16X3 && gemm_tile_override() == 0 && !a.ln_stat_in && a.N % 128 == 0 && gemm_sched_fuse_heuristic_pp(a, a.dtype == FDM_F32 ? 4 : 2);
    return pp ? FDM_TILE_256x128_PP : FDM_TILE_64x64;
  }
  const int want = gemm_tile_override();
  if (want > 0) return want;
  return gemm_heuristic_tile(a, a.dtype == FDM_F32 ? 4 : 2, a.dtype == FDM_F16X3);
}
}
```

face-diffusion-model_amd/csrc/kernels.hpp:

```cpp
#pragma once
#include <hip/hip_runtime.h>
#include "../../include/fdm_hip.h"

namespace fdm {
int fail(int code, const char* fmt, ...);
hipError_t gemm_launch_f32(const fdm_gemm_args& a, hipStream_t s);
hipError_t gemm_launch_bf16(const fdm_gemm_args& a, hipStream_t s);
hipError_t gemm_launch_f16x3(const fdm_gemm_args& a, hipStream_t s);
hipError_t gemm_launch_f16(const fdm_gemm_args& a, hipStream_t s);
int gemm_heuristic_tile_of(const fdm_gemm_args& a);
hipError_t attn_launch_f32(const fdm_attn_args& a, hipStream_t s);
hipError_t attn_launch_bf16(const fdm_attn_args& a, hipStream_t s);
hipError_t attn_launch_f16x3(const fdm_attn_args& a, hipStream_t s);
hipError_t attn_launch_f16(const fdm_attn_args& a, hipStream_t s);
hipError_t pack_kv_launch_f32(const void* K, long long ldk, const void* V, long long ldv, void* Kp, void* Vp, int B, int H, int L, int Lpad, int hd, hipStream_t s);
hipError_t pack_kv_launch_bf16(const void* K, long long ldk, const void* V, long long ldv, void* Kp, void* Vp, int B, int H, int L, int Lpad, int hd, hipStream_t s);

struct WinEnt { int w; int start; float wt; int pad; };
struct WinArgs {
  const int* off; const WinEnt* ent;
  float* xw;
  int L_total;
  int n_win;
  int W;
  int d;
  int init;
};
int window_sched_op(const fdm_sched_args& p, const WinArgs& w, void* stream);

int slot_advance_op(int* state, const int* tseq, int n_steps, int n_slots, void* stream);
int slot_set_op(int* state, int slot, int k, int t, int live, int run, unsigned long long* keys, unsigned long long seed, int clip_id, void* stream);
int slot_advance_bank_op(int* state, const fdm_slot_bank_args& b, int n_slots, void* stream);
int slot_set_bank_op(int* state, int slot, int k, int t, int live, int run, unsigned long long* keys, unsigned long long seed, int clip_id,
                     void* req, int sampler, float cfg_scale, void* stream);
int slot_park_op(int* state, int slot, void* stream);

struct LongFrame { int group; int e0; int e1; int pad; };
struct LongEnt { int slot; int start; float wt; int pad; };
struct LongGroup { int leader; int L_total; int first; int pad; };

inline hipError_t gemm_launch(const fdm_gemm_args& a, hipStream_t s) {
  switch (a.dtype) {
    case FDM_BF16: return gemm_launch_bf16(a, s);
    case FDM_F16X3: return gemm_launch_f16x3(a, s);
    case FDM_F16: return gemm_launch_f16(a, s);
    default: return gemm_launch_f32(a, s);
  }
}
inline hipError_t attn_launch(const fdm_attn_args& a, hipStream_t s) {
  return a.dtype == FDM_BF16 ? attn_launch_bf16(a, s) : (a.dtype == FDM_F16 ? attn_launch_f16(a, s) : (a.dtype == FDM_F16X3 ? attn_launch_f16x3(a, s) : attn_launch_f32(a, s)));
}
}
```

face-diffusion-model_amd/csrc/plan.hip:

```cpp
#include <hip/hip_runtime.h>

#include <cmath>
#include <cstdio>

#include "common.hpp"
#include "plan.hpp"

std::string fdm::shape_key(const fdm_plan* P) {
  char b[80];
  snprintf(b, sizeof(b), "%d,%d,%d,%d,%d,ks%d.%d", P->R, P->M, P->L, P->rep, P->S, P->ksplit_out, P->ksplit_ffn2);
  return b;
}

int fdm::drop_programs(fdm_plan* P, void* stream) {
  if (P->progs.empty()) return FDM_OK;
  if (stream) HIPCK(hipStreamSynchronize((hipStream_t)stream));
  else HIPCK(hipDeviceSynchronize());
  for (auto& kv : P->progs) fdm_prog_destroy(kv.second);
  P->progs.clear();
  P->prog_order.clear();
  P->pinned.clear();
  return FDM_OK;
}

namespace {
using namespace fdm;

__global__ void transpose_kernel(const float* in, float* out, int rows, int cols) {
  const long long n = (long long)rows * cols;
  for (long long i = (long long)blockIdx.x * blockDim.x + threadIdx.x; i < n; i += (long long)gridDim.x * blockDim.x) {
    const int c = (int)(i / rows), r = (int)(i % rows);
    out[i] = in[(size_t)r * cols + c];
  }
}
__global__ void scale_cols_kernel(const float* W, const float* gamma, float* out, long long n, int K) {
  for (long long i = (long long)blockIdx.x * blockDim.x + threadIdx.x; i < n; i += (long long)gridDim.x * blockDim.x)
    out[i] = W[i] * gamma[i % K];
}
__global__ __launch_bounds__(256) void rowsum_bf16_kernel(const fdm::bf16* W, float* out, int N, int K) {
  const int lane = threadIdx.x & 63, row = blockIdx.x * 4 + (threadIdx.x >> 6);
  if (row >= N) return;
  float s = 0.f;
  for (int k = lane; k < K; k += 64) s += (float)W[(size_t)row * K + k];
  s = fdm::wave_sum(s);
  if (lane == 0) out[row] = s;
}
template <typename E>
__global__ __launch_bounds__(256) void rowsum_split_kernel(const E* W, long long lo_off, float inv_scale, float* out, int N, int K) {
  const int lane = threadIdx.x & 63, row = blockIdx.x * 4 + (threadIdx.x >> 6);
  if (row >= N) return;
  float s = 0.f;
  for (int k = lane; k < K; k += 64) s += (float)W[(size_t)row * K + k] + (float)W[lo_off + (size_t)row * K + k] * inv_scale;
  s = fdm::wave_sum(s);
  if (lane == 0) out[row] = s;
}

template <typename T> int zalloc(Arena& a, T** out, size_t n) { return a.alloc_t(out, n, true); }
int zalloc_mat(const fdm_plan* P, Arena& a, Mat* out, size_t rows, size_t cols) {
  const size_t n = rows * cols;
  out->lo = kind(P->dtype).planes == 2 ? (long long)n : 0;
  return a.alloc(&out->p, n * kind(P->dtype).full(), true);
}

const Wt* weight(const fdm_plan* P, const std::string& name) {
  auto it = P->w.find(name);
  return it == P->w.end() ? nullptr : &it->second;
}
int need(const fdm_plan* P, const std::string& name, long long n, const float** out) { return need_weight(P->w, "plan: ", name, n, out); }

fdm_gemm_args gemm_op(const fdm_plan* P, const Mat& A, const Mat& W, int M, int N, int K) {
  fdm_gemm_args a = dense_gemm(P->dtype, A.p, W.p, M, N, K);
  a.a_lo_off = A.lo; a.w_lo_off = W.lo;
  return a;
}
void set_out_t(fdm_gemm_args& a, const Mat& o) { a.out_t = o.p; a.out_t_lo_off = o.lo; }

void set_ln_stats(fdm_gemm_args& g, const fdm_plan* P) { g.ln_stat_in = P->stats; g.ln_nparts = P->m.d / 64; g.ln_dim = P->m.d; g.ln_eps = 1e-5f; }
void set_ksplit(fdm_gemm_args& g, int S, long long plane) { if (S > 1) { g.ksplit = S; g.ksplit_stride = plane; } }
void set_ksplit(fdm_ln_args& ln, int S, long long plane) { if (S > 1) { ln.x_planes = S; ln.x_plane_stride = plane; } }

int plan_gemm(fdm_plan* P, const char* label, fdm_gemm_args a, void* stream) {
  if (P->tune_rec) (*P->tune_rec)[label].push_back(a);
  auto it = P->tiles.find(label);
  a.tile = (it == P->tiles.end() ? 0 : it->second) | (P->lockstep ? FDM_TILE_LOCKSTEP : 0);
  return fdm_op_gemm(&a, stream);
}

std::string lname(int l, const char* suffix) {
  char b[96];
  snprintf(b, sizeof(b), "transformer_decoder.layers.%d.%s", l, suffix);
  return b;
}

int commit_impl(fdm_plan* P, void* stream) {
  const fdm_model_desc& m = P->m;
  const int d = m.d;
  hipStream_t s = (hipStream_t)stream;
  FCK(drop_programs(P, stream));
  const float* p = nullptr;
  FCK(need(P, "audio_extract.0.weight", (long long)d * m.audio_in, &p));
  FCK(need(P, "audio_extract.0.bias", d, &p));
  FCK(need(P, "audio_extract.2.weight", (long long)d * d, &p));
  FCK(need(P, "audio_extract.2.bias", d, &p));
  FCK(need(P, "style_embedd.weight", (long long)d * m.n_style, &p));
  FCK(need(P, "style_embedd.bias", d, &p));
  if (m.n_emo) { FCK(need(P, "emotion_embedd.weight", (long long)d * m.n_emo, &p)); FCK(need(P, "emotion_embedd.bias", d, &p)); }
  FCK(need(P, "latent_encoder.0.bias", d, &p));
  FCK(need(P, "latent_decoder.bias", d, &p));
  std::vector<std::pair<std::string, long long>> mats = {{"latent_encoder.0.weight", (long long)d * d}, {"latent_decoder.weight", (long long)d * d}};
  for (int l = 0; l < m.n_layers; ++l) {
    mats.push_back({lname(l, "self_attn.in_proj_weight"), 3LL * d * d});
    mats.push_back({lname(l, "self_attn.out_proj.weight"), (long long)d * d});
    mats.push_back({lname(l, "linear1.weight"), (long long)m.ffn * d});
    mats.push_back({lname(l, "linear2.weight"), (long long)d * m.ffn});
    for (const char* b : {"self_attn.in_proj_bias", "self_attn.out_proj.bias", "linear1.bias", "linear2.bias", "norm1.weight", "norm1.bias",
                          "norm2.weight", "norm2.bias", "norm3.weight", "norm3.bias"}) {
      const long long nb = !strcmp(b, "self_attn.in_proj_bias") ? 3LL * d : (!strcmp(b, "linear1.bias") ? m.ffn : d);
      FCK(need(P, lname(l, b), nb, &p));
    }
  }
  for (auto& mt : mats) {
    FCK(need(P, mt.first, mt.second, &p));
    Mat o;
    FCK(to_operand(P->cmem, P->dtype, p, mt.second, &o, stream));
    P->wt[mt.first] = o;
  }
  const float *Wt_ = nullptr, *bt = nullptr;
  FCK(need(P, "time_embedd.0.weight", (long long)d * 1000, &Wt_));
  FCK(need(P, "time_embedd.0.bias", d, &bt));
  float* wtT = nullptr;
  FCK(zalloc(P->cmem, &wtT, (size_t)1000 * d));
  FCK(zalloc(P->cmem, &P->tau, (size_t)1000 * d));
  hipLaunchKernelGGL(transpose_kernel, dim3(grid_for(1000LL * d)), dim3(256), 0, s, Wt_, wtT, d, 1000);
  FCK(fdm_op_bias_act(wtT, bt, P->tau, 1000, d, FDM_ACT_MISH, stream));
  float* tmp = nullptr;
  FCK(zalloc(P->cmem, &tmp, (size_t)1000 * d));
  P->TT.assign(m.n_layers, nullptr);
  P->Wv.assign(m.n_layers, nullptr); P->bv = P->Wo = P->bo = P->Wv;
  for (int l = 0; l < m.n_layers; ++l) {
    const float *ipw = nullptr, *ipb = nullptr;
    FCK(need(P, lname(l, "multihead_attn.in_proj_weight"), 3LL * d * d, &ipw));
    FCK(need(P, lname(l, "multihead_attn.in_proj_bias"), 3LL * d, &ipb));
    FCK(need(P, lname(l, "multihead_attn.out_proj.weight"), (long long)d * d, &P->Wo[l]));
    FCK(need(P, lname(l, "multihead_attn.out_proj.bias"), d, &P->bo[l]));
    P->Wv[l] = ipw + 2LL * d * d;
    P->bv[l] = ipb + 2LL * d;
    FCK(zalloc(P->cmem, &P->TT[l], (size_t)1000 * d));
    fdm_gemm_args g = dense_gemm(FDM_F32, P->tau, P->Wv[l], 1000, d, d);
    g.out_f32 = tmp;
    FCK(fdm_op_gemm(&g, stream));
    g = dense_gemm(FDM_F32, tmp, P->Wo[l], 1000, d, d);
    g.out_f32 = P->TT[l];
    FCK(fdm_op_gemm(&g, stream));
  }
  P->fuse_ln3 = (P->dtype == FDM_BF16 || P->dtype == FDM_F16X3) && P->want_fuse_ln3;
  if (P->fuse_ln3) {
    auto make_fold = [&](const std::string& wname, const std::string& bname, int N, int l_prev, Fold* f) -> int {
      const float *W = nullptr, *b = nullptr, *gam = nullptr, *bet = nullptr;
      FCK(need(P, wname, (long long)N * d, &W));
      FCK(need(P, bname, N, &b));
      FCK(need(P, lname(l_prev, "norm3.weight"), d, &gam));
      FCK(need(P, lname(l_prev, "norm3.bias"), d, &bet));
      float* wg = nullptr;
      FCK(zalloc(P->cmem, &wg, (size_t)N * d));
      hipLaunchKernelGGL(scale_cols_kernel, dim3(grid_for((long long)N * d)), dim3(256), 0, s, W, gam, wg, (long long)N * d, d);
      FCK(to_operand(P->cmem, P->dtype, wg, (long long)N * d, &f->w, stream));
      FCK(zalloc(P->cmem, &f->colsum, (size_t)N));
// ... 157 lines not shown
    if (split) { at.q_lo_off = P->q_lo; at.kv_lo_off = P->kv_lo; at.o_lo_off = P->ctx.lo; }
    FCK(fdm_op_attention(&at, stream));
    FCK(need(P, lname(l, "self_attn.out_proj.bias"), d, &b));
    g = gemm_op(P, P->ctx, P->wt[lname(l, "self_attn.out_proj.weight")], R, d, d);
    g.bias = b; g.out_f32 = P->x1;
    if (!f) {
      g.resid = P->h;
      set_ksplit(g, P->ksplit_out, (long long)R * d);
      FCK(plan_gemm(P, "out", g, stream));
    } else {
      g.resid = P->x2; g.rln_gamma = f->gamma; g.rln_beta = f->beta; set_ln_stats(g, P);
      FCK(plan_gemm(P, "out_ln", g, stream));
    }
    fdm_ln_args ln;
    memset(&ln, 0, sizeof(ln));
    ln.x = P->x1; ln.M = R; ln.d = d; ln.add_mat = P->C1[l]; ln.add_tab = P->TT[l]; ln.tab_step = tcur; ln.eps = eps;
    if (P->S > 1) { ln.add_mat_L = L; ln.add_mat_group = P->S * L; ln.add_mat_wrap = M; }
    if (P->slots) {
      ln.tab_step = nullptr; ln.clip_step = P->slot_state + 1; ln.clip_step_stride = 4; ln.clip_rows = L; ln.clip_wrap = M;
    }
    if (!f) set_ksplit(ln, P->ksplit_out, (long long)R * d);
    FCK(need(P, lname(l, "norm1.weight"), d, &ln.gamma)); FCK(need(P, lname(l, "norm1.bias"), d, &ln.beta));
    FCK(need(P, lname(l, "norm2.weight"), d, &ln.gamma2)); FCK(need(P, lname(l, "norm2.bias"), d, &ln.beta2));
    ln.y_f32 = P->h2; ln.dtype = P->dtype;
    if (both) { ln.y_t = P->h2t.p; ln.y_t_lo_off = P->h2t.lo; }
    FCK(fdm_op_layernorm(&ln, stream));
    FCK(need(P, lname(l, "linear1.bias"), m.ffn, &b));
    g = gemm_op(P, P->h2t, P->wt[lname(l, "linear1.weight")], R, m.ffn, d);
    g.bias = b; g.act = FDM_ACT_RELU; set_out_t(g, P->u);
    FCK(plan_gemm(P, "ffn1", g, stream));
    FCK(need(P, lname(l, "linear2.bias"), d, &b));
    g = gemm_op(P, P->u, P->wt[lname(l, "linear2.weight")], R, d, m.ffn);
    g.bias = b; g.resid = P->h2;
    if (fuse) {
      g.out_f32 = P->x2; set_out_t(g, P->x2t); g.stat_out = P->stats;
      FCK(plan_gemm(P, "ffn2_stat", g, stream));
    } else {
      g.out_f32 = P->x1;
      set_ksplit(g, P->ksplit_ffn2, (long long)R * d);
      FCK(plan_gemm(P, "ffn2", g, stream));
      memset(&ln, 0, sizeof(ln));
      ln.x = P->x1; ln.M = R; ln.d = d; ln.eps = eps; ln.y_f32 = P->h; ln.dtype = P->dtype;
      set_ksplit(ln, P->ksplit_ffn2, (long long)R * d);
      FCK(need(P, lname(l, "norm3.weight"), d, &ln.gamma)); FCK(need(P, lname(l, "norm3.bias"), d, &ln.beta));
      if (both) { ln.y_t = P->ht.p; ln.y_t_lo_off = P->ht.lo; }
      FCK(fdm_op_layernorm(&ln, stream));
    }
  }
  fdm_gemm_args g;
  if (fuse) {
    const Fold& f = P->fold[-1];
    g = gemm_op(P, P->x2t, f.w, R, d, d);
    g.bias = f.bias; g.ln_colsum = f.colsum; set_ln_stats(g, P);
  } else {
    FCK(need(P, "latent_decoder.bias", d, &b));
    g = gemm_op(P, P->ht, P->wt["latent_decoder.weight"], R, d, d);
    g.bias = b;
  }
  if (sched) {
    g.resid = P->x; g.out_f32 = P->x;
    if (both) set_out_t(g, P->xt);
    g.sched_fuse = 1; g.sched = *sched;
  } else {
    g.out_f32 = P->x0;
  }
  return plan_gemm(P, fuse ? "dec_ln" : "dec", g, stream);
}

namespace {

struct ProgSpec {
  int kind;
  const float* noise = nullptr; float cfg_scale = 0.f;
  const float* san = nullptr; const float* cn = nullptr;
  int reps = 1;
  int slot_steps = 0;
  int bank = 0;
};

std::string tiles_sig(const fdm_plan* P) {
  std::string s;
  for (auto& kv : P->tiles)
    if (kv.second) s += kv.first + "=" + std::to_string(kv.second) + ",";
  s += "ks" + std::to_string(P->ksplit_out) + std::to_string(P->ksplit_ffn2) + (P->lockstep ? "L" : "");
  return s;
}

fdm::WinArgs win_args(const fdm_plan* P, int init) {
  fdm::WinArgs w;
  w.off = P->win_off; w.ent = P->win_ent; w.xw = P->x;
  w.L_total = P->win_total; w.n_win = P->win_n; w.W = P->win_len; w.d = P->m.d; w.init = init;
  return w;
}

fdm_slot_group_args long_args(const fdm_plan* P, int f0, int f1, int plain, int init) {
  fdm_slot_group_args g;
  memset(&g, 0, sizeof(g));
  g.member = P->slot_member; g.frames = (const int*)P->long_frame; g.entries = P->long_ent; g.groups = (const int*)P->long_group;
  g.x_long = P->long_x; g.hist_long = P->long_hist;
  g.arena_frames = P->long_frames; g.n_entries = P->long_entries; g.n_groups = P->long_groups;
  g.L = P->L; g.d = P->m.d; g.frame0 = f0; g.frame1 = f1; g.plain = plain; g.init = init;
  return g;
}

fdm_slot_bank_args bank_args(const fdm_plan* P) {
  fdm_slot_bank_args b;
  memset(&b, 0, sizeof(b));
  b.req = P->slot_req; b.desc = P->bank_desc; b.t = P->bank_t; b.coef = P->bank_c;
  b.n_samplers = P->bank_rows; b.n_t = P->bank_t_cap; b.n_coef = P->bank_c_cap;
  return b;
}

int get_program(fdm_plan* P, const ProgSpec& sp, void* stream, fdm_prog** out) {
  char key[512];
  snprintf(key, sizeof(key), "%s#%s|%d|%p|%a|%p|%d", shape_key(P).c_str(), tiles_sig(P).c_str(), sp.kind, (const void*)sp.noise, (double)sp.cfg_scale,
           (const void*)sp.san, sp.reps);
  if (P->win_n) {
    const size_t kl = strlen(key);
    snprintf(key + kl, sizeof(key) - kl, "|win%d,%d,%d,%d,%d", P->win_B, P->win_total, P->win_n, P->win_len, P->win_overlap);
  }
  if (P->slots) {
    const size_t kl = strlen(key);
    snprintf(key + kl, sizeof(key) - kl, "|slot%d,%d,%p", sp.slot_steps, P->slots, (const void*)sp.cn);
    if (P->long_frames) {
      const size_t k2 = strlen(key);
      snprintf(key + k2, sizeof(key) - k2, "|long%d,%d", P->long_frames, P->long_groups);
    }
    if (sp.bank) {
      const size_t k3 = strlen(key);
      snprintf(key + k3, sizeof(key) - k3, "|bank%d,%d,%d", P->bank_rows, P->bank_t_cap, P->bank_c_cap);
    }
  }
  auto it = P->progs.find(key);
  if (it != P->progs.end()) {
    auto pos = std::find(P->prog_order.begin(), P->prog_order.end(), std::string(key));
    if (pos != P->prog_order.end()) { P->prog_order.erase(pos); P->prog_order.push_back(key); }
    P->pinned.push_back(key);
    if (sp.reps == 1) P->launches_per_step = fdm_prog_num_ops(it->second);
    *out = it->second;
    return FDM_OK;
  }
  if (P->progs.size() >= 16) {
    auto victim = P->prog_order.end();
    for (auto v = P->prog_order.begin(); v != P->prog_order.end(); ++v)
      if (std::find(P->pinned.begin(), P->pinned.end(), *v) == P->pinned.end()) { victim = v; break; }
    if (victim != P->prog_order.end()) {
      HIPCK(hipStreamSynchronize((hipStream_t)stream));
      const std::string vk = *victim;
      P->prog_order.erase(victim);
      fdm_prog_destroy(P->progs[vk]);
      P->progs.erase(vk);
    }
  }
  const int d = P->m.d, M = P->M;
  const long long n = (long long)M * d;
  fdm_prog* prog = nullptr;
  FCK(fdm_prog_create(&prog));
  int rc = fdm_prog_begin(prog);
  const bool fuse_sched = !P->cfg && sp.kind != 0 && !sp.slot_steps;
  for (int rep = 0; rc == FDM_OK && rep < sp.reps; ++rep) {
    fdm_sched_args sc;
    memset(&sc, 0, sizeof(sc));
    sc.x0 = P->x0; sc.x0u = P->cfg ? P->x0 + n : nullptr; sc.cfg_scale = sp.cfg_scale;
    sc.x = P->x; sc.x_out = P->x; sc.n = n; sc.tseq = P->tseq; sc.step = P->step; sc.advance = 0;
    if (P->dtype != FDM_F32) { sc.x_out_t = P->xt.p; sc.out_dtype = P->dtype; sc.x_out_t_lo_off = P->xt.lo; }
    if (sp.kind == 1) {
      sc.mode = 0; sc.n_per_clip = (long long)P->L * d; sc.c1 = P->c1; sc.c2 = P->c2; sc.sigma = P->sigma;
// ... 858 lines not shown
  g = fdm_plan::GroupHost();
  return FDM_OK;
}

int fdm_slot_sampler_add(fdm_plan* P, const fdm_sample_args* a, void* stream) {
  if (!a) return fail(FDM_ERR_ARG, "slot_sampler_add: null sampler");
  if (a->noise || a->record) return fail(FDM_ERR_ARG, "slot_sampler_add: injected noise and record are not supported in slot mode");
  if (!P) return fail(FDM_ERR_ARG, "slot_sampler_add: null plan");
  FCK(check_slots(P, "slot_sampler_add"));
  SamplerDef def;
  FCK(sampler_def(a, "slot_sampler_add", def));
  if (!P->bank_rows) return fail(FDM_ERR_STATE, "slot_sampler_add: the session has no sampler bank (fdm_plan_set slot_samplers / slot_sampler_steps before fdm_slots_open)");
  int id = -1;
  for (int i = 1; i < P->bank_rows && id < 0; ++i)
    if (!P->sampler_host[i].used) id = i;
  if (id < 0) return fail(FDM_ERR_STATE, "slot_sampler_add: all %d bank rows are in use", P->bank_rows - 1);
  auto first_fit = [&](bool coef, int need, int cap) {
    std::vector<std::pair<int, int>> used;
    for (const auto& h : P->sampler_host)
      if (h.used && (coef ? h.n_c : h.n_steps) > 0) used.push_back(coef ? std::make_pair(h.c_off, h.n_c) : std::make_pair(h.t_off, h.n_steps));
    std::sort(used.begin(), used.end());
    int at = 0;
    for (const auto& u : used) {
      if (u.first - at >= need) return at;
      at = u.first + u.second;
    }
    return cap - at >= need ? at : -1;
  };
  const int nt = (int)def.ts.size(), nc = (int)def.coef.size();
  const int t_off = first_fit(false, nt, P->bank_t_cap), c_off = nc ? first_fit(true, nc, P->bank_c_cap) : 0;
  if (t_off < 0) return fail(FDM_ERR_STATE, "slot_sampler_add: no free range of %d timesteps (bank %d)", nt, P->bank_t_cap);
  if (c_off < 0) return fail(FDM_ERR_STATE, "slot_sampler_add: no free range of %d coefficients (bank %d)", nc, P->bank_c_cap);
  hipStream_t s = (hipStream_t)stream;
  const int desc[4] = {def.mode, nt, t_off, c_off};
  HIPCK(hipMemcpyAsync(P->bank_t + t_off, def.ts.data(), (size_t)nt * 4, hipMemcpyHostToDevice, s));
  if (nc) HIPCK(hipMemcpyAsync(P->bank_c + c_off, def.coef.data(), (size_t)nc * 4, hipMemcpyHostToDevice, s));
  HIPCK(hipMemcpyAsync(P->bank_desc + 4 * (size_t)id, desc, 16, hipMemcpyHostToDevice, s));
  HIPCK(hipStreamSynchronize(s));
  fdm_plan::SamplerHost& h = P->sampler_host[id];
  h.used = true; h.kind = def.kind; h.mode = def.mode; h.n_steps = nt; h.t0 = def.ts[0]; h.t_off = t_off; h.c_off = c_off; h.n_c = nc;
  return id;
}

int fdm_slot_sampler_drop(fdm_plan* P, int id) {
  if (!P) return fail(FDM_ERR_ARG, "slot_sampler_drop: null plan");
  FCK(check_slots(P, "slot_sampler_drop"));
  if (id < 1 || id >= P->bank_rows || !P->sampler_host[id].used) return fail(FDM_ERR_ARG, "slot_sampler_drop: %s", id == 0 ? "sampler 0 belongs to the session" : "unknown sampler");
  for (size_t i = 0; i < P->slot_host.size(); ++i)
    if (P->slot_host[i].status != 0 && P->slot_host[i].sampler == id)
      return fail(FDM_ERR_STATE, "slot_sampler_drop: slot %d (%s) names sampler %d", (int)i, P->slot_host[i].status == 1 ? "running" : "finished and not read", id);
  P->sampler_host[id] = fdm_plan::SamplerHost();
  return FDM_OK;
}

int fdm_slot_sampler_info(fdm_plan* P, int id, int* kind, int* n_steps) {
  if (!P) return fail(FDM_ERR_ARG, "slot_sampler_info: null plan");
  FCK(check_slots(P, "slot_sampler_info"));
  if (!P->bank_rows) {
    if (id != 0) return fail(FDM_ERR_ARG, "slot_sampler_info: unknown sampler %d", id);
    if (kind) *kind = P->slot_kind - 1;
    if (n_steps) *n_steps = P->slot_nsteps;
    return FDM_OK;
  }
  if (id < 0 || id >= P->bank_rows || !P->sampler_host[id].used) return fail(FDM_ERR_ARG, "slot_sampler_info: unknown sampler %d", id);
  if (kind) *kind = P->sampler_host[id].kind;
  if (n_steps) *n_steps = P->sampler_host[id].n_steps;
  return FDM_OK;
}

int fdm_plan_tune(fdm_plan* P, void* stream) {
  FCK(check_ready(P));
  return tune_tiles(P, 1, stream);
}

int fdm_plan_get(fdm_plan* P, const char* key, long long* out) {
  if (!P || !key || !out) return fail(FDM_ERR_ARG, "plan_get: null argument");
  const std::string k(key);
  if (k == "launches_per_step") *out = P->launches_per_step;
  else if (k == "graph_launches") *out = P->last_graph_launches;
  else if (k == "fuse_ln3") *out = P->fuse_ln3;
  else if (k == "rows") *out = P->R;
  else if (k == "ksplit.out") *out = P->ksplit_out;
  else if (k == "ksplit.ffn2") *out = P->ksplit_ffn2;
  else if (k == "tuned") *out = P->tile_cache.count(shape_key(P)) ? 1 : 0;
  else if (k == "needs_tune") *out = needs_tune(P, shape_key(P)) ? 1 : 0;
  else if (k == "tune_failed") *out = P->tune_failed;
  else if (k == "windows") *out = P->win_n;
  else if (k == "slots") *out = P->slots;
  else if (k == "slot_long_frames") *out = P->want_long_frames;
  else if (k == "slot_long_groups") *out = P->want_long_groups;
  else if (k == "slot_samplers") *out = P->want_samplers;
  else if (k == "slot_sampler_steps") *out = P->want_sampler_steps;
  else if (k == "window_len") *out = P->win_n ? P->win_len : P->L;
  else if (k == "L_total") *out = P->win_n ? P->win_total : P->L;
  else if (k.rfind("tile.", 0) == 0) { auto it = P->tiles.find(k.substr(5)); *out = it == P->tiles.end() ? 0 : it->second; }
  else return fail(FDM_ERR_ARG, "plan_get: unknown key '%s'", key);
  return FDM_OK;
}

int fdm_plan_set(fdm_plan* P, const char* key, long long value) {
  if (!P || !key) return fail(FDM_ERR_ARG, "plan_set: null argument");
  const std::string k(key);
  if (k == "tune") { P->tune_enabled = value != 0; return FDM_OK; }
  if (k == "tune_lazy") { P->tune_lazy = value != 0; return FDM_OK; }
  if (k == "slot_long_frames" || k == "slot_long_groups") {
    if (value < 0 || value > 0x3fffffffLL) return fail(FDM_ERR_ARG, "plan_set: %s = %lld", key, value);
    (k == "slot_long_frames" ? P->want_long_frames : P->want_long_groups) = (int)value;
    return FDM_OK;
  }
  if (k == "slot_samplers" || k == "slot_sampler_steps") {
    if (value < 0 || value > 0xfffffLL) return fail(FDM_ERR_ARG, "plan_set: %s = %lld", key, value);
    (k == "slot_samplers" ? P->want_samplers : P->want_sampler_steps) = (int)value;
    return FDM_OK;
  }
  if (k == "fuse_ln3") {
    if ((value != 0) != (P->want_fuse_ln3 != 0)) { P->want_fuse_ln3 = value != 0; P->committed = false; P->prepared = false; return drop_programs(P, nullptr); }
    return FDM_OK;
  }
  if (k == "ksplit.out" || k == "ksplit.ffn2") {
    const int kt = (k == "ksplit.out" ? P->m.d : P->m.ffn) / kind(P->dtype).bk;
    if (value < 1 || value > 4 || kt % value) return fail(FDM_ERR_ARG, "plan_set: %s = %lld must be 1..4 and divide the %d k-tiles", key, value, kt);
    int& cur = k == "ksplit.out" ? P->ksplit_out : P->ksplit_ffn2;
    if (cur == (int)value) return FDM_OK;
    cur = (int)value;
    P->tile_cache.clear(); P->tiles.erase(k == "ksplit.out" ? "out" : "ffn2");
    FCK(drop_programs(P, nullptr));
    if (P->capB > 0 && (int)value > P->x1_planes) {
      P->x1_planes = (int)value;
      FCK(zalloc(P->ws, &P->x1, (size_t)P->capB * P->capL * P->capRep * P->m.d * P->x1_planes));
    }
    return FDM_OK;
  }
  if (k == "lockstep") { P->lockstep = value != 0; P->tile_cache.clear(); P->tiles.clear(); return drop_programs(P, nullptr); }
  if (k == "untune") {
    P->tile_cache.clear(); P->steps_seen.clear(); P->tiles.clear(); P->tune_failed_shapes.clear();
    return drop_programs(P, nullptr);
  }
  if (k.rfind("tile.", 0) == 0) {
    if (value < 0 || value > FDM_TILE_MAX) return fail(FDM_ERR_ARG, "plan_set: unknown tile %lld", value);
    P->tiles[k.substr(5)] = (int)value;
    P->tile_cache[shape_key(P)] = P->tiles;
    return drop_programs(P, nullptr);
  }
  return fail(FDM_ERR_ARG, "plan_set: unknown key '%s'", key);
}

}
```

face-diffusion-model_amd/csrc/plan.hpp:

```cpp
#pragma once
#include <set>

#include "host.hpp"

struct Fold { fdm::Mat w; float* colsum = nullptr; float* bias = nullptr; const float* gamma = nullptr; const float* beta = nullptr; };

struct fdm_plan {
  fdm_model_desc m{};
  int dtype = FDM_F32, hd = 0;
  fdm::Arena mem, ws, cmem;
  std::map<std::string, fdm::Wt> w;
  bool committed = false;
  std::map<std::string, fdm::Mat> wt;
  float* tau = nullptr;
  std::vector<float*> TT;
  std::vector<const float*> Wv, bv, Wo, bo;
  bool fuse_ln3 = false;
  std::map<int, Fold> fold;
  float *slopes = nullptr, *pe = nullptr;
  float *c1 = nullptr, *c2 = nullptr, *sigma = nullptr, *sra = nullptr, *srm1 = nullptr;
  int capB = 0, capL = 0, capRep = 0;
  int B = 0, L = 0, M = 0, rep = 1, R = 0, Lpad = 0, cfg = 0;
  int S = 1;
  bool prepared = false;
  float *h = nullptr, *h2 = nullptr, *x1 = nullptr, *x0 = nullptr, *x = nullptr, *x2 = nullptr, *stats = nullptr;
  fdm::Mat xt, ht, h2t, x2t, ctx, u;
  void *q = nullptr, *kp = nullptr, *vp = nullptr;
  long long q_lo = 0, kv_lo = 0;
  size_t kv_bytes = 0;
  float *AF = nullptr, *t1 = nullptr, *sty = nullptr, *em = nullptr, *emu = nullptr, *zeros = nullptr, *E0 = nullptr;
  std::vector<float*> C1;
  int* step = nullptr;
  unsigned long long* seedbuf = nullptr;
  int* tseq = nullptr; int tseq_cap = 0;
  float* lm_tab = nullptr; int lm_cap = 0;
  float* x0_hist = nullptr;
  std::map<int, std::pair<int, float*>> ddim;
  std::map<int, std::vector<int>> ddim_t;
  std::map<std::string, fdm_prog*> progs;
  std::vector<std::string> prog_order;
  std::vector<std::string> pinned;
  std::map<std::string, int> tiles;
  std::map<std::string, std::map<std::string, int>> tile_cache;
  std::map<std::string, long long> steps_seen;
  std::map<std::string, std::vector<fdm_gemm_args>>* tune_rec = nullptr;
  int tune_enabled = 1;
  int tune_failed = 0;
  std::set<std::string> tune_failed_shapes;
  int want_fuse_ln3 = 0;
  int ksplit_out = 1, ksplit_ffn2 = 1;
  int x1_planes = 0;
  int lockstep = 0;
  int tune_lazy = 0;
  long long last_graph_launches = 0, launches_per_step = 0;
  int win_n = 0, win_len = 0, win_total = 0, win_overlap = 0, win_B = 0;
  float* xlong = nullptr; size_t xlong_cap = 0;
  float* hist_long = nullptr; size_t hist_long_cap = 0;
  int* win_off = nullptr; size_t win_off_cap = 0;
  fdm::WinEnt* win_ent = nullptr; size_t win_ent_cap = 0;
  float* win_stage = nullptr; size_t win_stage_cap = 0;
  int slots = 0;
  int* slot_state = nullptr; size_t slot_state_cap = 0;
  unsigned long long* slot_keys = nullptr; size_t slot_keys_cap = 0;
  struct SlotHost { int status = 0, done = 0, L = 0, group = -1, sampler = 0, total = 0; };
  std::vector<SlotHost> slot_host;
  int slot_kind = 0, slot_nsteps = 0, slot_t0 = 0;
  int slot_graph_steps = 0, slot_eager = 0;
  float slot_cfg_scale = 0.f;
  const float *slot_san = nullptr, *slot_cn = nullptr;
  int want_long_frames = 0, want_long_groups = 0;
  int long_frames = 0, long_groups = 0, long_entries = 0;
  float* long_x = nullptr; size_t long_x_cap = 0;
  float* long_hist = nullptr; size_t long_hist_cap = 0;
  fdm::LongFrame* long_frame = nullptr; size_t long_frame_cap = 0;
  fdm::LongEnt* long_ent = nullptr; size_t long_ent_cap = 0;
  fdm::LongGroup* long_group = nullptr; size_t long_group_cap = 0;
  int* slot_member = nullptr; size_t slot_member_cap = 0;
  struct GroupHost { bool used = false; int L_total = 0, first = 0, e0 = 0, ne = 0; std::vector<int> slots; };
  std::vector<GroupHost> group_host;
  int want_samplers = 0, want_sampler_steps = 0;
  int bank_rows = 0, bank_t_cap = 0, bank_c_cap = 0;
  void* slot_req = nullptr; size_t slot_req_cap = 0;
  int* bank_desc = nullptr; size_t bank_desc_cap = 0;
  int* bank_t = nullptr; size_t bank_t_bytes = 0;
  float* bank_c = nullptr; size_t bank_c_bytes = 0;
  struct SamplerHost { bool used = false; int kind = 0, mode = 0, n_steps = 0, t0 = 0, t_off = 0, c_off = 0, n_c = 0; };
  std::vector<SamplerHost> sampler_host;
};

namespace fdm {
std::string shape_key(const fdm_plan* P);
int drop_programs(fdm_plan* P, void* stream);
int record_chain(fdm_plan* P, const fdm_sched_args* sched, void* stream);
bool needs_tune(fdm_plan* P, const std::string& key);
int tune_tiles(fdm_plan* P, int force, void* stream);
void tune_soft(fdm_plan* P, void* stream);
void select_tiles(fdm_plan* P);
}
```

face-diffusion-model_amd/csrc/tune.hip:

```cpp
#include <cstdio>
#include <cstdlib>
#include <fstream>

#include <unistd.h>

#include "plan.hpp"

namespace {
using namespace fdm;

int time_prog(fdm_prog* prog, int warm, int reps, hipStream_t s, float* ms) {
  hipEvent_t e0, e1;
  HIPCK(hipEventCreate(&e0)); HIPCK(hipEventCreate(&e1));
  int rc = fdm_prog_instantiate(prog, s);
  if (rc == FDM_OK) rc = fdm_prog_replay(prog, warm, s);
  if (rc == FDM_OK) {
    (void)hipEventRecord(e0, s);
    rc = fdm_prog_replay(prog, reps, s);
    (void)hipEventRecord(e1, s);
    (void)hipEventSynchronize(e1);
    (void)hipEventElapsedTime(ms, e0, e1);
  }
  (void)hipEventDestroy(e0); (void)hipEventDestroy(e1);
  return rc;
}

std::vector<std::pair<std::string, int>> parse_tiles(const std::string& v) {
  std::vector<std::pair<std::string, int>> out;
  size_t pos = 0;
  while (pos < v.size()) {
    const size_t comma = v.find(',', pos), eq = v.find('=', pos);
    const size_t end = comma == std::string::npos ? v.size() : comma;
    if (eq != std::string::npos && eq < end) out.push_back({v.substr(pos, eq - pos), atoi(v.substr(eq + 1, end - eq - 1).c_str())});
    pos = end + 1;
  }
  return out;
}

void apply_tile_override(std::map<std::string, int>& tiles) {
  if (const char* ov = getenv("FDM_TILE_OVERRIDE"))
    for (auto& kv : parse_tiles(ov)) tiles[kv.first] = kv.second;
}

std::string store_key(const fdm_plan* P) {
  const fdm_model_desc& m = P->m;
  char b[160];
  snprintf(b, sizeof(b), "v%d|dt%d|%d,%d,%d,%d,%d,%d,%d,%d|%s", fdm_version(), P->dtype, m.d, m.n_head, m.n_layers, m.ffn, m.G, m.c, m.audio_in, m.pair,
           shape_key(P).c_str());
  return b;
}

bool store_read(std::map<std::string, std::string>& lines) {
  const char* path = getenv("FDM_TILE_CACHE");
  if (!path || !*path) return false;
  std::ifstream f(path);
  std::string ln;
  while (f && std::getline(f, ln)) {
    const size_t tab = ln.find('\t');
    if (tab != std::string::npos) lines[ln.substr(0, tab)] = ln.substr(tab + 1);
  }
  return true;
}

bool store_lookup(const fdm_plan* P, std::map<std::string, int>& tiles) {
  std::map<std::string, std::string> lines;
  if (!store_read(lines)) return false;
  auto it = lines.find(store_key(P));
  if (it == lines.end()) return false;
  tiles.clear();
  for (auto& kv : parse_tiles(it->second)) {
    if (kv.second < 0 || kv.second > FDM_TILE_MAX) return false;
    if (kv.second) tiles[kv.first] = kv.second;
  }
  return true;
}

void store_save(const fdm_plan* P, const std::map<std::string, int>& tiles) {
  std::map<std::string, std::string> lines;
  if (!store_read(lines)) return;
  std::string v;
  for (auto& kv : tiles)
    if (kv.second) v += (v.empty() ? "" : ",") + kv.first + "=" + std::to_string(kv.second);
  lines[store_key(P)] = v;
  const std::string path = getenv("FDM_TILE_CACHE"), tmp = path + ".tmp" + std::to_string((long long)getpid());
  {
    std::ofstream f(tmp, std::ios::trunc);
    if (!f) return;
    for (auto& kv : lines) f << kv.first << '\t' << kv.second << '\n';
  }
  if (rename(tmp.c_str(), path.c_str()) != 0) remove(tmp.c_str());
}

bool tuning_on(const fdm_plan* P) {
  const char* env = getenv("FDM_TUNE");
  return P->tune_enabled && !(env && !strcmp(env, "0"));
}

int tune_tiles_impl(fdm_plan* P, void* stream) {
  const std::string key = shape_key(P);
  hipStream_t s = (hipStream_t)stream;
  const Kind& kd = kind(P->dtype);
  const bool split = kd.planes == 2;
  FCK(drop_programs(P, stream));
  P->tiles.clear();
  std::map<std::string, std::vector<fdm_gemm_args>> calls;
  {
    fdm_prog* dry = nullptr;
    FCK(fdm_prog_create(&dry));
    int rc = fdm_prog_begin(dry);
    P->tune_rec = &calls;
    if (rc == FDM_OK) rc = record_chain(P, nullptr, stream);
    P->tune_rec = nullptr;
    (void)fdm_prog_end(dry);
    fdm_prog_destroy(dry);
    FCK(rc);
  }
  auto timed = [&](const std::vector<fdm_gemm_args>& inst, int tile, float* best) -> int {
    *best = 1e30f;
    for (int rep = 0; rep < 3; ++rep) {
      fdm_prog* prog = nullptr;
      FCK(fdm_prog_create(&prog));
      int rc = fdm_prog_begin(prog);
      for (size_t i = 0; rc == FDM_OK && i < inst.size(); ++i) { fdm_gemm_args a = inst[i]; a.tile = tile | (P->lockstep ? FDM_TILE_LOCKSTEP : 0); a.incr_counter = nullptr; a.incr_table = nullptr; rc = fdm_op_gemm(&a, stream); }
      (void)fdm_prog_end(prog);
      float ms = 0.f;
      if (rc == FDM_OK) rc = time_prog(prog, 2, 5, s, &ms);
      HIPCK(hipStreamSynchronize(s));
      fdm_prog_destroy(prog);
      FCK(rc);
      if (ms < *best) *best = ms;
    }
    return FDM_OK;
  };
  std::vector<int> cands = {FDM_TILE_64x64, FDM_TILE_64x64_S2, FDM_TILE_32x64_S3, FDM_TILE_128x64, FDM_TILE_128x128, FDM_TILE_80x128, FDM_TILE_64x128};
  if (!split && P->R >= 1024) cands.push_back(FDM_TILE_256x128_PP);
  struct Geo { int bm, bn, nst; };
  auto geo = [&](int tile) -> Geo {
    switch (tile) {
      case FDM_TILE_64x64_S2: return {64, 64, 2};
      case FDM_TILE_32x64_S3: return {32, 64, 3};
      case FDM_TILE_128x64: return {128, 64, split ? 3 : 4};
      case FDM_TILE_128x128: return {128, 128, split ? 2 : 3};
      case FDM_TILE_80x128: return {80, 128, split ? 3 : 4};
      case FDM_TILE_64x128: return {64, 128, split ? 3 : 4};
      case FDM_TILE_256x128_PP: return {256, 128, 3};
      default: return {64, 64, 4};
    }
  };
  auto modelled_us = [&](const fdm_gemm_args& a, int tile) {
    const Geo g = geo(tile);
    const double planes = kd.planes, eb = kd.bytes;
    const long long tiles = (long long)((a.M + g.bm - 1) / g.bm) * ((a.N + g.bn - 1) / g.bn) * (a.batch > 0 ? a.batch : 1);
    const long long rounds = (tiles + 255) / 256;
    const double bytes = (double)rounds * (g.bm + g.bn) * a.K * eb * planes;
    return 5.0 + bytes / 70e3;
  };
  std::map<std::string, int> tuned, runner_up;
  for (auto& kv : calls) {
    std::vector<fdm_gemm_args> inst = kv.second;
    while (inst.size() < 4) { auto c = inst; inst.insert(inst.end(), c.begin(), c.end()); }
    float base = 0.f;
    FCK(timed(inst, 0, &base));
    std::vector<std::pair<float, int>> cand = {{base * 0.97f, 0}};
    double best_model = 1e30;
    for (int tile : cands) best_model = std::min(best_model, modelled_us(kv.second[0], tile));
    auto launched = [&](int tile) {
      if (!split) return tile;
      return tile == FDM_TILE_256x128_PP ? FDM_TILE_128x128 : tile;
    };
    const int heur = launched(fdm_gemm_heuristic_tile(&kv.second[0]));
    for (int tile : cands) {
      if (launched(tile) == heur) continue;
      if (kv.second[0].ksplit > 1 && tile != FDM_TILE_64x64 && tile != FDM_TILE_64x64_S2 && tile != FDM_TILE_32x64_S3) continue;
      if (kv.second[0].sched_fuse && tile != FDM_TILE_256x128_PP && tile != FDM_TILE_64x64) continue;
      if (modelled_us(kv.second[0], tile) > 1.35 * best_model) continue;
      float t = 0.f;
      FCK(timed(inst, tile, &t));
      cand.push_back({t, tile});
    }
    std::sort(cand.begin(), cand.end());
    tuned[kv.first] = cand[0].second;
    if (cand.size() > 1 && cand[1].first < cand[0].first * 1.05f) runner_up[kv.first] = cand[1].second;
  }
  auto chain_time = [&](const std::map<std::string, int>& tiles, float* best) -> int {
    *best = 1e30f;
    for (int rep = 0; rep < 2; ++rep) {
      P->tiles = tiles;
      const int init[2] = {-1, 0};
      HIPCK(hipMemcpyAsync(P->step, init, 8, hipMemcpyHostToDevice, s));
      fdm_prog* prog = nullptr;
      FCK(fdm_prog_create(&prog));
      int rc = fdm_prog_begin(prog);
      if (rc == FDM_OK) rc = record_chain(P, nullptr, stream);
      (void)fdm_prog_end(prog);
      float ms = 0.f;
      if (rc == FDM_OK) rc = time_prog(prog, 2, 4, s, &ms);
      HIPCK(hipStreamSynchronize(s));
      fdm_prog_destroy(prog);
      FCK(rc);
      if (ms < *best) *best = ms;
    }
    return FDM_OK;
  };
  bool any = !runner_up.empty();
  for (auto& kv : tuned) any = any || kv.second != 0;
  std::map<std::string, int> keep;
  if (any) {
    float t_h = 0.f, t_t = 0.f;
    FCK(chain_time({}, &t_h));
    FCK(chain_time(tuned, &t_t));
    for (auto& kv : runner_up) {
      std::map<std::string, int> trial = tuned;
      trial[kv.first] = kv.second;
      float t_a = 0.f;
      FCK(chain_time(trial, &t_a));
      if (t_a < 0.997f * t_t) { tuned = trial; t_t = t_a; }
    }
    if (t_t < 0.99f * t_h) {
      float t_h2 = 0.f;
      FCK(chain_time({}, &t_h2));
      t_h = std::min(t_h, t_h2);
    }
    if (t_t < 0.99f * t_h) keep = tuned;
    if (getenv("FDM_TUNE_VERBOSE")) {
      std::string desc;
      for (auto& kv : tuned) desc += kv.first + "=" + std::to_string(kv.second) + ",";
      fprintf(stderr, "[fdm tune] rows=%d candidates: %s chain %.3f -> %.3f ms: %s\n", P->R, desc.c_str(), t_h / 4, t_t / 4, keep.empty() ? "rejected" : "kept");
    }
  }
  P->tiles = keep;
  apply_tile_override(P->tiles);
  P->tile_cache[key] = P->tiles;
  return FDM_OK;
}

}

bool fdm::needs_tune(fdm_plan* P, const std::string& key) {
  return !P->tile_cache.count(key) && tuning_on(P) && P->steps_seen.count(key) && P->steps_seen[key] >= 2000 && !P->tune_failed_shapes.count(key);
}

int fdm::tune_tiles(fdm_plan* P, int force, void* stream) {
  const std::string key = shape_key(P);
  if (P->tile_cache.count(key) || !tuning_on(P)) return FDM_OK;
  if (!force && !needs_tune(P, key)) return FDM_OK;
  const std::map<std::string, int> before = P->tiles;
  const int rc = tune_tiles_impl(P, stream);
  if (rc != FDM_OK) { P->tiles = before; (void)drop_programs(P, stream); if (!force) P->tune_failed_shapes.insert(key); }
  else { store_save(P, P->tiles); P->tune_failed_shapes.erase(key); }
  return rc;
}

void fdm::tune_soft(fdm_plan* P, void* stream) {
  if (tune_tiles(P, 0, stream) != FDM_OK) ++P->tune_failed;
}

void fdm::select_tiles(fdm_plan* P) {
// ... 15 lines not shown
```

face-diffusion-model_amd/fdm_amd/_lib.py:

```python
import ctypes as C
import os

_HERE = os.path.dirname(os.path.abspath(__file__))
LIB_PATH = os.environ.get("FDM_LIB_PATH") or os.path.join(_HERE, "libfdm_hip.so")

F32, BF16, F16X3, F16 = 0, 1, 2, 3
DTYPE_NAMES = {"f32": F32, "bf16": BF16, "f16x3": F16X3, "f16": F16}
SAMPLER_DPMPP_2M, SAMPLER_DDIM = 0, 1
SLOT_IDLE, SLOT_RUNNING, SLOT_FINISHED = 0, 1, 2
SAMPLER_NAMES = {"dpmpp2m": SAMPLER_DPMPP_2M, "ddim_eta": SAMPLER_DDIM}
ACT_NONE, ACT_RELU, ACT_MISH, ACT_GELU_ERF, ACT_GELU_TANH, ACT_LEAKY02 = range(6)

vp, ll, ci, cf = C.c_void_p, C.c_longlong, C.c_int, C.c_float


class SchedArgs(C.Structure):
    _fields_ = [("x0", vp), ("x0u", vp), ("cfg_scale", cf), ("x", vp), ("x_out", vp),
                ("n", ll), ("n_per_clip", ll), ("tseq", vp), ("step", vp), ("advance", ci),
                ("c1", vp), ("c2", vp), ("sigma", vp), ("sra", vp), ("srm1", vp),
                ("sqrt_an", vp), ("c_n", vp), ("noise", vp), ("noise_stride", ll), ("x_out_t", vp), ("out_dtype", ci), ("arrive", vp),
                ("seed", C.c_ulonglong), ("clip0", ci),
                ("mode", ci), ("x_out_t_lo_off", ll), ("seed_dev", vp),
                ("lm_a", vp), ("lm_b", vp), ("lm_c", vp), ("lm_s", vp), ("x0_hist", vp)]


class GemmArgs(C.Structure):
    _fields_ = [("A", vp), ("lda", ll), ("a_batch_stride", ll),
                ("W", vp), ("ldw", ll), ("w_batch_stride", ll),
                ("M", ci), ("N", ci), ("K", ci), ("batch", ci), ("dtype", ci),
                ("bias", vp), ("bias_batch_stride", ll), ("act", ci),
                ("resid", vp), ("ldr", ll), ("resid_row_mod", ci),
                ("out_f32", vp), ("ldo_f32", ll), ("out_t", vp), ("ldo_t", ll),
                ("out_batch_stride", ll),
                ("out_kp", vp), ("kp_col0", ci), ("out_vp", vp), ("vp_col0", ci),
                ("kv_L", ci), ("kv_Lpad", ci), ("kv_hd", ci),
                ("stat_out", vp), ("ln_stat_in", vp), ("ln_nparts", ci), ("ln_dim", ci), ("ln_eps", cf),
                ("ln_colsum", vp), ("rln_gamma", vp), ("rln_beta", vp), ("incr_counter", vp), ("incr_table", vp), ("tile", ci),
                ("sched_fuse", ci), ("sched", SchedArgs),
                ("a_lo_off", ll), ("w_lo_off", ll), ("out_t_lo_off", ll), ("kv_lo_off", ll),
                ("ksplit", ci), ("ksplit_stride", ll), ("batch2", ci), ("a_batch_stride2", ll), ("out_batch_stride2", ll)]


TILE_AUTO, TILE_64x64, TILE_128x64, TILE_128x128, TILE_64x64_S2, TILE_32x64_S3, TILE_256x128_PP, TILE_80x128, TILE_64x128 = 0, 1, 2, 3, 8, 9, 10, 11, 12
TILE_96x128, TILE_256x128, TILE_64x64_S3, TILE_128x64_S3 = 4, 5, 6, 7


class ModelDesc(C.Structure):
    _fields_ = [(n, ci) for n in ("d", "n_head", "n_layers", "ffn", "G", "c", "n_style", "n_emo", "audio_in", "pair",
                                  "pe_periodic", "period", "latent_mish", "style_mish", "max_len")]


class SampleArgs(C.Structure):
    _fields_ = [("kind", ci), ("x_T", vp), ("out", vp), ("t_list", vp), ("n_steps", ci), ("ddim_steps", ci), ("noise", vp),
                ("seed", C.c_ulonglong), ("clip0", ci), ("cfg_scale", cf), ("eager", ci), ("record", vp), ("graph_steps", ci),
                ("lm_tables", vp)]


class VqDesc(C.Structure):
    _fields_ = [(n, ci) for n in ("G", "c", "K", "n_books", "V3", "pre")]


class AttnArgs(C.Structure):
    _fields_ = [("Q", vp), ("ldq", ll), ("Kp", vp), ("Vp", vp), ("Lpad", ci),
                ("O", vp), ("ldo", ll), ("B", ci), ("H", ci), ("L", ci), ("hd", ci), ("dtype", ci),
                ("scale", cf), ("causal", ci), ("slopes", vp), ("period", ci), ("o_split", ci), ("o_lo_off", ll), ("q_lo_off", ll), ("kv_lo_off", ll),
                ("lens", vp)]


class LnArgs(C.Structure):
    _fields_ = [("x", vp), ("M", ci), ("d", ci), ("add_mat", vp), ("add_tab", vp),
                ("tab_index", vp), ("tab_step", vp), ("gamma", vp), ("beta", vp), ("eps", cf),
                ("act", ci), ("y_f32", vp), ("y_t", vp), ("dtype", ci), ("gamma2", vp), ("beta2", vp), ("y_t_lo_off", ll),
                ("add_mat_L", ci), ("add_mat_group", ci), ("add_mat_wrap", ci), ("x_planes", ci), ("x_plane_stride", ll),
                ("clip_step", vp), ("clip_step_stride", ci), ("clip_rows", ci), ("clip_wrap", ci)]


class SlotGroupArgs(C.Structure):
    _fields_ = [("member", vp), ("frames", vp), ("entries", vp), ("groups", vp), ("x_long", vp), ("hist_long", vp),
                ("arena_frames", ci), ("n_entries", ci), ("n_groups", ci), ("L", ci), ("d", ci), ("frame0", ci), ("frame1", ci),
                ("plain", ci), ("init", ci)]


class SlotBankArgs(C.Structure):
    _fields_ = [("req", vp), ("desc", vp), ("t", vp), ("coef", vp), ("n_samplers", ci), ("n_t", ci), ("n_coef", ci), ("reserved", ci)]


STRUCTS = {"fdm_sched_args": SchedArgs, "fdm_gemm_args": GemmArgs, "fdm_attn_args": AttnArgs, "fdm_ln_args": LnArgs,
           "fdm_model_desc": ModelDesc, "fdm_sample_args": SampleArgs, "fdm_vq_desc": VqDesc, "fdm_slot_group_args": SlotGroupArgs,
           "fdm_slot_bank_args": SlotBankArgs}

SYMBOLS = {
    "fdm_last_error": (C.c_char_p, []),
    "fdm_version": (ci, []),
    "fdm_abi_struct_size": (ci, [C.c_char_p]),
    "fdm_device_ok": (ci, []),
    "fdm_op_gemm": (ci, [C.POINTER(GemmArgs), vp]),
    "fdm_gemm_heuristic_tile": (ci, [C.POINTER(GemmArgs)]),
    "fdm_op_attention": (ci, [C.POINTER(AttnArgs), vp]),
    "fdm_op_pack_kv": (ci, [vp, ll, vp, ll, vp, vp, ci, ci, ci, ci, ci, ci, vp]),
    "fdm_op_layernorm": (ci, [C.POINTER(LnArgs), vp]),
    "fdm_op_sched_step": (ci, [C.POINTER(SchedArgs), vp]),
    "fdm_op_slot_sched": (ci, [C.POINTER(SchedArgs), vp, vp, ci, vp]),
    "fdm_op_slot_group_sched": (ci, [C.POINTER(SchedArgs), vp, vp, ci, C.POINTER(SlotGroupArgs), vp]),
    "fdm_op_slot_sched_bank": (ci, [C.POINTER(SchedArgs), vp, vp, ci, C.POINTER(SlotBankArgs), vp]),
    "fdm_op_slot_group_sched_bank": (ci, [C.POINTER(SchedArgs), vp, vp, ci, C.POINTER(SlotGroupArgs), C.POINTER(SlotBankArgs), vp]),
    "fdm_op_cast": (ci, [vp, vp, ll, ci, vp]),
    "fdm_op_vertex_err": (ci, [vp, vp, vp, ci, ci, ci, vp, vp, vp, vp]),
    "fdm_op_motion_std": (ci, [vp, vp, vp, ci, ci, ci, vp, vp, vp]),
    "fdm_op_linear_interp": (ci, [vp, vp, ci, ci, ci, ci, vp]),
    "fdm_op_bias_act": (ci, [vp, vp, vp, ll, ci, ci, vp]),
    "fdm_op_add_rows": (ci, [vp, ci, ci, vp, ci, ci, vp, ci, ci, vp, ll, ci, vp]),
    "fdm_op_small_linear": (ci, [vp, vp, vp, vp, ci, ci, ci, ci, vp]),
    "fdm_op_pad_rows": (ci, [vp, vp, ci, ci, ci, ci, ci, ci, vp]),
    "fdm_op_pad_rows_lens": (ci, [vp, vp, ci, ci, ci, ci, ci, vp, vp]),
    "fdm_op_zero_pad_rows": (ci, [vp, ci, ci, ci, vp, vp]),
    "fdm_op_group_pad": (ci, [vp, vp, ci, ci, ci, ci, ci, ci, vp]),
    "fdm_op_set_ints": (ci, [vp, vp, ci, vp]),
    "fdm_op_mask_samples": (ci, [vp, vp, ci, ci, vp, vp]),
    "fdm_op_group_pad_lens": (ci, [vp, vp, ci, ci, ci, ci, ci, ci, vp, vp]),
    "fdm_op_conv0": (ci, [vp, vp, vp, vp, ci, ci, ci, vp]),
    "fdm_op_conv0_ln_gelu": (ci, [vp, vp, vp, vp, vp, vp, ll, ci, ci, ci, cf, ci, vp]),
    "fdm_op_leaky_instnorm": (ci, [vp, vp, vp, ci, ci, ci, cf, ci, vp]),
    "fdm_op_leaky_instnorm_lens": (ci, [vp, vp, vp, ci, ci, ci, cf, ci, vp, vp]),
    "fdm_op_adain": (ci, [vp, vp, vp, ci, ci, ci, cf, vp]),
    "fdm_op_mean_diff": (ci, [vp, vp, vp, vp, ll, ci, vp]),
    "fdm_op_time_groupnorm": (ci, [vp, vp, vp, vp, vp, ll, ci, ci, ci, cf, ci, ci, vp, ll, vp]),
    "fdm_op_time_groupnorm_lens": (ci, [vp, vp, vp, vp, vp, ll, ci, ci, ci, cf, ci, ci, vp, ll, vp, vp]),
# ... 100 lines not shown
```

include/fdm_hip.h:

```cpp
#ifndef FDM_HIP_H
#define FDM_HIP_H

#ifdef __cplusplus
extern "C" {
#endif

#define FDM_F32 0
#define FDM_BF16 1
#define FDM_F16X3 2
#define FDM_F16 3

#define FDM_ACT_NONE 0
#define FDM_ACT_RELU 1
#define FDM_ACT_MISH 2
#define FDM_ACT_GELU_ERF 3
#define FDM_ACT_GELU_TANH 4
#define FDM_ACT_LEAKY02 5

#define FDM_OK 0
#define FDM_ERR_ARG (-1)
#define FDM_ERR_SHAPE (-2)
#define FDM_ERR_HIP (-3)
#define FDM_ERR_STATE (-4)

// ... 7 lines not shown
  const float* x; float* x_out;
  long long n; long long n_per_clip;
  const int* tseq; int* step; int advance;
  const float* c1; const float* c2; const float* sigma;
  const float* sra; const float* srm1;
  const float* sqrt_an; const float* c_n;
  const float* noise; long long noise_stride;
  void* x_out_t; int out_dtype;
  unsigned int* arrive;
  unsigned long long seed; int clip0;
  int mode;
  long long x_out_t_lo_off;
  const unsigned long long* seed_dev;
  const float* lm_a; const float* lm_b; const float* lm_c; const float* lm_s;
  float* x0_hist;
} fdm_sched_args;
int fdm_op_sched_step(const fdm_sched_args* a, void* stream);
int fdm_op_slot_sched(const fdm_sched_args* a, const int* state, const unsigned long long* keys, int n_slots, void* stream);
typedef struct fdm_slot_group_args {
  const int* member; const int* frames; const void* entries; const int* groups;
  float* x_long; float* hist_long;
  int arena_frames, n_entries, n_groups;
  int L, d;
  int frame0, frame1;
  int plain, init;
} fdm_slot_group_args;
int fdm_op_slot_group_sched(const fdm_sched_args* a, const int* state, const unsigned long long* keys, int n_slots,
                            const fdm_slot_group_args* g, void* stream);
typedef struct fdm_slot_bank_args {
  const void* req; const int* desc; const int* t; const float* coef;
  int n_samplers, n_t, n_coef;
  int reserved;
} fdm_slot_bank_args;
int fdm_op_slot_sched_bank(const fdm_sched_args* a, const int* state, const unsigned long long* keys, int n_slots,
                           const fdm_slot_bank_args* b, void* stream);
int fdm_op_slot_group_sched_bank(const fdm_sched_args* a, const int* state, const unsigned long long* keys, int n_slots,
                                 const fdm_slot_group_args* g, const fdm_slot_bank_args* b, void* stream);

typedef struct fdm_gemm_args {
  const void* A; long long lda; long long a_batch_stride;
  const void* W; long long ldw; long long w_batch_stride;
  int M, N, K, batch;
  int dtype;
  const float* bias; long long bias_batch_stride;
  int act;
  const float* resid; long long ldr; int resid_row_mod;
  float* out_f32; long long ldo_f32;
  void* out_t; long long ldo_t;
  long long out_batch_stride;
  void* out_kp; int kp_col0;
  void* out_vp; int vp_col0;
  int kv_L; int kv_Lpad; int kv_hd;
  float* stat_out;
  const float* ln_stat_in; int ln_nparts; int ln_dim; float ln_eps;
  const float* ln_colsum;
  const float* rln_gamma; const float* rln_beta;
  int* incr_counter;
  const int* incr_table;
  int tile;
  int sched_fuse;
  fdm_sched_args sched;
  long long a_lo_off, w_lo_off, out_t_lo_off;
  long long kv_lo_off;
  int ksplit; long long ksplit_stride;
  int batch2; long long a_batch_stride2, out_batch_stride2;
} fdm_gemm_args;
#define FDM_TILE_AUTO 0
#define FDM_TILE_64x64 1
#define FDM_TILE_128x64 2
#define FDM_TILE_128x128 3
#define FDM_TILE_64x64_S2 8
#define FDM_TILE_32x64_S3 9
#define FDM_TILE_256x128_PP 10
#define FDM_TILE_80x128 11
#define FDM_TILE_64x128 12
#define FDM_TILE_96x128 4
#define FDM_TILE_256x128 5
#define FDM_TILE_64x64_S3 6
#define FDM_TILE_128x64_S3 7
#define FDM_TILE_MAX 12
#define FDM_TILE_GENERAL 0x100
#define FDM_TILE_LOCKSTEP 0x200
#define FDM_TILE_ID_MASK 0xff
int fdm_op_gemm(const fdm_gemm_args* a, void* stream);
int fdm_gemm_heuristic_tile(const fdm_gemm_args* a);

typedef struct fdm_attn_args {
  const void* Q; long long ldq;
  const void* Kp;
  const void* Vp; int Lpad;
  void* O; long long ldo;
  int B, H, L, hd;
  int dtype;
  float scale;
  int causal;
  const float* slopes;
  int period;
  int o_split; long long o_lo_off;
  long long q_lo_off, kv_lo_off;
  const int* lens;
} fdm_attn_args;
int fdm_op_attention(const fdm_attn_args* a, void* stream);
int fdm_op_pack_kv(const void* K, long long ldk, const void* V, long long ldv, void* Kp, void* Vp,
                   int B, int H, int L, int Lpad, int hd, int dtype, void* stream);

typedef struct fdm_ln_args {
  const float* x; int M, d;
  const float* add_mat;
  const float* add_tab;
  const int* tab_index; const int* tab_step;
  const float* gamma; const float* beta; float eps;
  int act;
  float* y_f32; void* y_t; int dtype;
  const float* gamma2; const float* beta2;
  long long y_t_lo_off;
  int add_mat_L, add_mat_group, add_mat_wrap;
  int x_planes; long long x_plane_stride;
  const int* clip_step; int clip_step_stride, clip_rows, clip_wrap;
} fdm_ln_args;
int fdm_op_layernorm(const fdm_ln_args* a, void* stream);


int fdm_op_cast(const float* src, void* dst, long long n, int dtype, void* stream);
int fdm_op_bias_act(const float* in, const float* vec, float* out, long long rows, int d, int act, void* stream);
int fdm_op_add_rows(const float* a, int a_div, int a_mod, const float* b, int b_div, int b_mod,
                    const float* c, int c_div, int c_mod, float* out, long long M, int d, void* stream);
int fdm_op_small_linear(const float* x, const float* W, const float* bias, float* out, int B, int K, int d,
                        int act, void* stream);
int fdm_op_pad_rows(const void* in, void* out, int B, int L, int d, int pad, int dtype, int zero, void* stream);
int fdm_op_pad_rows_lens(const void* in, void* out, int B, int L, int d, int pad, int dtype, const int* lens, void* stream);
int fdm_op_zero_pad_rows(float* x, int B, int L, int d, const int* lens, void* stream);
int fdm_op_set_ints(int* dst, const int* src, int n, void* stream);
int fdm_op_mask_samples(const float* wav, float* out, int B, int n, const int* lens, void* stream);
int fdm_op_group_pad_lens(const void* in, void* out, int B, int T, int d, int groups, int pad, int dtype, const int* lens, void* stream);
int fdm_op_conv0(const float* wav, const float* w, const float* bias, float* out, int B, int n, int T0, void* stream);
int fdm_op_conv0_ln_gelu(const float* wav, const float* w, const float* bias, const float* gamma, const float* beta, void* out,
                         long long out_lo_off, int B, int n, int T0, float eps, int dtype, void* stream);
int fdm_op_leaky_instnorm(const float* x, float* y_f32, void* y_t, int B, int L, int d, float eps, int dtype, void* stream);
int fdm_op_leaky_instnorm_lens(const float* x, float* y_f32, void* y_t, int B, int L, int d, float eps, int dtype, const int* lens, void* stream);
int fdm_op_time_groupnorm(const float* x, const float* gamma, const float* beta, float* y_f32, void* y_t, long long y_t_lo_off, int B, int T, int C,
                          float eps, int act, int dtype, void* scratch, long long scratch_bytes, void* stream);
int fdm_op_time_groupnorm_lens(const float* x, const float* gamma, const float* beta, float* y_f32, void* y_t, long long y_t_lo_off, int B, int T, int C,
                               float eps, int act, int dtype, void* scratch, long long scratch_bytes, const int* lens, void* stream);
int fdm_op_mean_diff(const float* a, const float* b, float* partial, float* out, long long n, int l1, void* stream);
int fdm_op_vertex_err(const float* gt, const float* pred, const int* region, int R, int F, int V,
                      float* frame_max, double* frame_sum, double* out, void* stream);
int fdm_op_motion_std(const float* verts, const float* tmpl, const int* region, int R, int F, int V,
                      double* partial, double* out, void* stream);
int fdm_op_linear_interp(const float* x, float* y, int B, int Tin, int Tout, int C, void* stream);
int fdm_op_adain(const float* content, const float* style, float* out, int NC, int Lc, int Ls, float eps, void* stream);
int fdm_op_group_pad(const void* in, void* out, int B, int T, int d, int groups, int pad, int dtype, void* stream);

int fdm_op_vq_quant(const float* z, const float* codebook, const int* book, int B, int R, int c, int K,
                    float* zq_bcl, long long* idx, void* stream);
int fdm_op_vq_stats(const float* z, const float* codebook, const int* book, const long long* idx, int B, int R, int c, int K, float beta,
                    float* min_encodings, double* partial, int* hist, float* out, void* stream);

typedef struct fdm_prog fdm_prog;
int fdm_prog_create(fdm_prog** out);
int fdm_prog_destroy(fdm_prog* p);
int fdm_prog_begin(fdm_prog* p);
int fdm_prog_end(fdm_prog* p);
int fdm_prog_run(fdm_prog* p, void* stream);
int fdm_prog_instantiate(fdm_prog* p, void* stream);
int fdm_prog_replay(fdm_prog* p, int n, void* stream);
int fdm_prog_num_ops(fdm_prog* p);
// ... 104 lines not shown
```

Baseline: 2012 frames/s.

## Add row-pitch GEMM tiles that spread short-M problems across more workgroups

Adds a row pitch encoded in the tile bits. A 64-row tile then covers only `pitch` live rows (below 64), so small-M GEMMs launch more row blocks and fill more CUs. Loads, vmcnt waits and the epilogue are masked to the live rows. The autotuner gets pitched candidates, and the heuristic proposes a pitch only when the FDM_ROW_PITCH env var is set. The cost is wasted MFMA work on the dead rows and more redundant weight reads.

```diff
diff --git a/face-diffusion-model_amd/csrc/fdm_hip.hip b/face-diffusion-model_amd/csrc/fdm_hip.hip
--- a/face-diffusion-model_amd/csrc/fdm_hip.hip
+++ b/face-diffusion-model_amd/csrc/fdm_hip.hip
@@ -116,6 +116,8 @@
   if (a->rln_gamma && (!a->rln_beta || !a->resid)) return fail(FDM_ERR_ARG, "gemm: rln_gamma needs rln_beta and resid");
   if ((a->stat_out || a->ln_stat_in) && (a->batch > 1 || a->out_batch_stride)) return fail(FDM_ERR_ARG, "gemm: LayerNorm folding is not batched");
   if (a->tile < 0 || (a->tile & FDM_TILE_ID_MASK) > FDM_TILE_MAX) return fail(FDM_ERR_ARG, "gemm: unknown tile %d", a->tile);
+  if ((a->tile & ~(FDM_TILE_ID_MASK | FDM_TILE_GENERAL | FDM_TILE_LOCKSTEP | FDM_TILE_NO_PITCH | (FDM_TILE_PITCH_MASK << FDM_TILE_PITCH_SHIFT))) || FDM_TILE_PITCH(a->tile) > 64)
+    return fail(FDM_ERR_ARG, "gemm: unknown bits or a row pitch above 64 in tile 0x%x", a->tile);
   if (a->sched_fuse) {
     const fdm_sched_args& sc = a->sched;
     if (sc.mode != 0 && sc.mode != 1 && sc.mode != 3) return fail(FDM_ERR_ARG, "gemm: fused scheduler supports mode 0 (DDPM), 1 (DDIM) and 3 (table-driven)");
@@ -160,7 +162,7 @@
 
 int fdm_gemm_heuristic_tile(const fdm_gemm_args* a) {
   if (!a) return fail(FDM_ERR_ARG, "gemm_heuristic_tile: null argument");
-  return fdm::gemm_heuristic_tile_of(*a);
+  return fdm::gemm_heuristic_tile_of(*a) & FDM_TILE_ID_MASK;
 }
 
 int fdm_op_attention(const fdm_attn_args* a, void* stream) {
diff --git a/face-diffusion-model_amd/csrc/gemm.hpp b/face-diffusion-model_amd/csrc/gemm.hpp
--- a/face-diffusion-model_amd/csrc/gemm.hpp
+++ b/face-diffusion-model_amd/csrc/gemm.hpp
@@ -44,12 +44,12 @@
 
 template <int MI, int NI> struct EpiPre { f32x4 csv[NI], bv[NI], gmv[NI], btv[NI], rv[MI][NI]; SchedCoef sc; };
 
-template <typename T, int BM, int BN, int WM, int WN, int SCHED = 0>
+template <typename T, int BM, int BN, int WM, int WN, int SCHED = 0, bool PITCH = false>
 __device__ __forceinline__ void gemm_epi_preload(const fdm_gemm_args& p, int m0, int n0, int z, int wm, int wn, int g, int r16,
-                                                 bool ln_capable, EpiPre<BM / WM / 16, BN / WN / 16>& e) {
+                                                 bool ln_capable, EpiPre<BM / WM / 16, BN / WN / 16>& e, int row_end = 0) {
   constexpr int MI = BM / WM / 16, NI = BN / WN / 16;
   if constexpr (SCHED != 0) e.sc = sched_coef_load<SCHED == 2>(p.sched);
-  const int M = p.M, N = p.N;
+  const int M = PITCH ? row_end : p.M, N = p.N;
   const bool use_ln = ln_capable && p.ln_stat_in;
   const float* bias = p.bias ? p.bias + (size_t)z * p.bias_batch_stride : nullptr;
   const size_t ocol = (size_t)z * p.out_batch_stride;
@@ -92,7 +92,7 @@
 }
 __host__ __device__ inline bool gemm_act_is_heavy(int act) { return act == ACT_MISH || act == ACT_GELU_ERF || act == ACT_GELU_TANH; }
 
-constexpr int GEMM_LEAN = 1, GEMM_KV = 2, GEMM_FOLD = 4, GEMM_KSPLIT = 8, GEMM_B2 = 16, GEMM_LM = 32;
+constexpr int GEMM_LEAN = 1, GEMM_KV = 2, GEMM_FOLD = 4, GEMM_KSPLIT = 8, GEMM_B2 = 16, GEMM_LM = 32, GEMM_PITCH = 64;
 template <int MODE> struct KSliceArgs;
 template <> struct KSliceArgs<0> {
   const fdm_gemm_args& a;
@@ -117,15 +117,16 @@
 template <typename T, int BM, int BN, int WM = 2, int WN = 2, bool HEAVY = true, bool SCHED = false, int SPEC = 0>
 __device__ __forceinline__ void gemm_epilogue(const fdm_gemm_args& p, f32x4 (&acc)[BM / WM / 16][BN / WN / 16],
                                               const EpiPre<BM / WM / 16, BN / WN / 16>& e, int m0, int n0, int z,
-                                              int wm, int wn, int g, int r16, float* rowstat = nullptr, char* tile_lds = nullptr) {
+                                              int wm, int wn, int g, int r16, float* rowstat = nullptr, char* tile_lds = nullptr, int row_end = 0) {
   constexpr int MI = BM / WM / 16, NI = BN / WN / 16;
   constexpr bool LEAN = (SPEC & GEMM_LEAN) != 0;
+  static_assert(!(SPEC & GEMM_PITCH) || (LEAN && !(SPEC & (GEMM_KV | GEMM_FOLD | GEMM_KSPLIT | GEMM_B2))), "row pitch: lean forms only");
   constexpr bool KVC = !LEAN || (SPEC & GEMM_KV), FOLDC = !LEAN || (SPEC & GEMM_FOLD);
   using E = typename Opnd<T>::E;
   using KK = typename Opnd<T>::KV;
   using KV = typename Opnd<KK>::E;
   constexpr int KNP = Opnd<KK>::NP;
-  const int M = p.M, N = p.N;
+  const int M = (SPEC & GEMM_PITCH) ? row_end : p.M, N = p.N;
   constexpr int EPC_T = 16 / (int)sizeof(KV);
   const bool vt_tile = KVC && tile_lds && p.out_vp && n0 >= p.vp_col0 && n0 + BN <= N && (p.kv_L % EPC_T == 0);
   KV* tl = (KV*)tile_lds;
@@ -373,6 +374,8 @@
   constexpr bool UNEVEN = NA % IW != 0;
   static_assert(NWP % IW == 0 && BM % RPI == 0 && MI >= 1 && NI >= 1, "tile does not fit the wave grid");
   constexpr int A_IPW = (NA + IW - 1) / IW, W_IPW = NWP / IW;
+  constexpr bool PITCH = (SPEC & GEMM_PITCH) != 0;
+  static_assert(!PITCH || (!UNEVEN && A_IPW <= 2 && KCH == 8), "row pitch: tiles whose A pieces divide evenly, one or two per issuing wave");
   constexpr int P = NP * (A_IPW + W_IPW), P_LO = NP * (A_IPW - 1 + W_IPW);
   constexpr int STAGE = NP * (BM + BN) * ROWB;
   static_assert(NST * STAGE >= gemm_epi_ring_bytes<T, BM, BN>(), "epilogue staging does not fit in the ring");
@@ -412,10 +415,12 @@
     const int r2 = r - c2 * ny * nx;
     by = r2 / nx; bx = r2 - by * nx;
   }
-  const int m0 = by * BM, n0 = bx * BN;
+  const int pitch = PITCH ? (int)((unsigned)pK >> 24) : BM;
+  const int m0 = by * pitch, n0 = bx * BN;
   const int M = pM, N = pN;
+  const int live = PITCH ? min(pitch, M - m0) : BM;
   constexpr int EPC = 16 / (int)sizeof(E);
-  int nk = pK / (KCH * EPC);
+  int nk = (PITCH ? (pK & 0xffffff) : pK) / (KCH * EPC);
   const E* A = (const E*)pA;
   const E* W = (const E*)pW;
   if (z) {
@@ -446,6 +451,16 @@
     const int row = RPI * (wave * W_IPW + i) + lrow;
     w_src[i] = (const char*)(W + (size_t)min(n0 + row, N - 1) * p_ldw) + ((slot ^ (row % KCH)) << 4);
   }
+  int a_cnt = A_IPW;
+  bool a_lane[A_IPW];
+  if constexpr (PITCH) {
+    a_cnt = 0;
+#pragma unroll
+    for (int i = 0; i < A_IPW; ++i) {
+      a_cnt += (RPI * (wave * A_IPW + i) < live) ? 1 : 0;
+      a_lane[i] = RPI * (wave * A_IPW + i) + lrow < live;
+    }
+  }
   auto issue = [&](int kt) {
     char* sb = smem + (kt % NST) * STAGE;
     const size_t off = (size_t)kt * ROWB;
@@ -453,7 +468,12 @@
     for (int pl = 0; pl < NP; ++pl) {
 #pragma unroll
       for (int i = 0; i < A_IPW; ++i) {
-        if constexpr (UNEVEN) {
+        if constexpr (PITCH) {
+          if (i < a_cnt) {
+            if (a_lane[i])
+              __builtin_amdgcn_global_load_lds((gptr_t)(a_src[i] + off + pl * a_lo), (lptr_t)(sb + pl * BM * ROWB + (wave * A_IPW + i) * 1024), 16, 0, 0);
+          }
+        } else if constexpr (UNEVEN) {
           if (i * IW + wave < NA)
             __builtin_amdgcn_global_load_lds((gptr_t)(a_src[i] + off + pl * a_lo), (lptr_t)(sb + pl * BM * ROWB + (i * IW + wave) * 1024), 16, 0, 0);
         } else {
@@ -466,6 +486,16 @@
     }
   };
 
+  auto wait_tile = [&]() {
+    if constexpr (PITCH) {
+      if (a_cnt == A_IPW) wait_vmcnt<(NST - 2) * P>();
+      else if (A_IPW == 2 && a_cnt == 1) wait_vmcnt<(NST - 2) * NP * (1 + W_IPW)>();
+      else wait_vmcnt<(NST - 2) * NP * W_IPW>();
+    } else {
+      if (!UNEVEN || wave < NA % IW) wait_vmcnt<(NST - 2) * P>();
+      else wait_vmcnt<(NST - 2) * P_LO>();
+    }
+  };
   f32x4 acc[MI][NI];
   f32x4 accl[NP == 2 ? MI : 1][NP == 2 ? NI : 1];
 #pragma unroll
@@ -490,8 +520,7 @@
     if (loader) {
       for (int kt = 0; kt < nk; ++kt) {
         if (kt + NST - 2 < nk) {
-          if (!UNEVEN || wave < NA % IW) wait_vmcnt<(NST - 2) * P>();
-          else wait_vmcnt<(NST - 2) * P_LO>();
+          wait_tile();
         } else {
           wait_vmcnt<0>();
         }
@@ -503,7 +532,8 @@
   }
   EpiPre<MI, NI> epre;
   constexpr bool FOLDC = !(SPEC & GEMM_LEAN) || (SPEC & GEMM_FOLD);
-  gemm_epi_preload<T, BM, BN, WM, WN, (SCHED ? ((SPEC & GEMM_LM) ? 2 : 1) : 0)>(pe, m0, n0, z, wm, wn, g, r16, FOLDC, epre);
+  const int row_end = m0 + live;
+  gemm_epi_preload<T, BM, BN, WM, WN, (SCHED ? ((SPEC & GEMM_LM) ? 2 : 1) : 0), PITCH>(pe, m0, n0, z, wm, wn, g, r16, FOLDC, epre, row_end);
   if constexpr (FOLDC) gemm_load_rowstats<BM>(p, m0, rowstat);
 
   auto frag_a = [&](const char* base, int pl, int s, int mi) {
@@ -527,8 +557,7 @@
   for (int kt = 0; kt < nk; ++kt) {
     if constexpr (LW == 0) {
       if (kt + NST - 2 < nk) {
-        if (!UNEVEN || wave < NA % IW) wait_vmcnt<(NST - 2) * P>();
-        else wait_vmcnt<(NST - 2) * P_LO>();
+        wait_tile();
       } else {
         wait_vmcnt<0>();
       }
@@ -593,12 +622,12 @@
 #endif
   if constexpr (LW > 0) wait_vmcnt<0>();
 #ifndef FDM_GEMM_STAMPS
-  gemm_epilogue<T, BM, BN, WM, WN, HEAVY, SCHED, SPEC>(pe, acc, epre, m0, n0, z, wm, wn, g, r16, rowstat, smem);
+  gemm_epilogue<T, BM, BN, WM, WN, HEAVY, SCHED, SPEC>(pe, acc, epre, m0, n0, z, wm, wn, g, r16, rowstat, smem, row_end);
 #else
   const int passes = (stamps && p.sched.advance == 2 && !SCHED) ? 2 : 1;
 #pragma clang loop unroll(disable)
   for (int pass = 0; pass < passes; ++pass) {
-    gemm_epilogue<T, BM, BN, WM, WN, HEAVY, SCHED, SPEC>(pe, acc, epre, m0, n0, z, wm, wn, g, r16, rowstat, smem);
+    gemm_epilogue<T, BM, BN, WM, WN, HEAVY, SCHED, SPEC>(pe, acc, epre, m0, n0, z, wm, wn, g, r16, rowstat, smem, row_end);
     if (stamps && tid == 0) stamps[pass == 0 ? 3 : 6] = wall_clock64();
     asm volatile("s_waitcnt vmcnt(0)" ::: "memory");
     __syncthreads();
@@ -839,7 +868,8 @@
 
 template <typename T, int BM, int BN, int WM, int WN, int NST, int KCH, bool HEAVY, bool SCHED = false, int SPEC = 0, int LW = 0>
 static hipError_t gemm_glds_launch_h(const fdm_gemm_args& a, hipStream_t s) {
-  dim3 grid((a.N + BN - 1) / BN, (a.M + BM - 1) / BM, (SPEC & GEMM_KSPLIT) ? a.ksplit : (a.batch > 0 ? a.batch : 1) * ((SPEC & GEMM_B2) ? a.batch2 : 1));
+  const int pitch = (SPEC & GEMM_PITCH) ? FDM_TILE_PITCH(a.tile) : BM;
+  dim3 grid((a.N + BN - 1) / BN, (a.M + pitch - 1) / pitch, (SPEC & GEMM_KSPLIT) ? a.ksplit : (a.batch > 0 ? a.batch : 1) * ((SPEC & GEMM_B2) ? a.batch2 : 1));
   constexpr int lds = NST * Opnd<T>::NP * (BM + BN) * KCH * 16 + gemm_ln_scratch_bytes<BM, BN>();
   static_assert(lds <= 160 * 1024, "ring does not fit the CU's LDS");
   static bool once = [] {
@@ -847,7 +877,8 @@
   }();
   (void)once;
   hipLaunchKernelGGL((gemm_glds_kernel<T, BM, BN, WM, WN, NST, KCH, HEAVY, SCHED, SPEC, LW>), grid, dim3(64 * (WM * WN + LW)), lds, s,
-                     a.A, a.W, (long long)a.a_lo_off, (long long)a.w_lo_off, a.M, a.N, a.K, (int)a.lda, (int)a.ldw, a);
+                     a.A, a.W, (long long)a.a_lo_off, (long long)a.w_lo_off, a.M, a.N, (SPEC & GEMM_PITCH) ? (int)((unsigned)a.K | ((unsigned)pitch << 24)) : a.K,
+                     (int)a.lda, (int)a.ldw, a);
   return hipGetLastError();
 }
 static bool gemm_lockstep_env() {
@@ -855,10 +886,10 @@
   return v;
 }
 template <typename T, int BM, int BN>
-static bool gemm_all_tiles_lean(const fdm_gemm_args& a) {
+static bool gemm_all_tiles_lean(const fdm_gemm_args& a, bool row_mod_ok = false) {
   using E = typename Opnd<T>::E;
   auto al = [](const void* p, size_t n) { return ((uintptr_t)p % n) == 0; };
-  if (a.N % BN || a.out_batch_stride % 4 || a.resid_row_mod) return false;
+  if (a.N % BN || a.out_batch_stride % 4 || (a.resid_row_mod && !row_mod_ok)) return false;
   if (a.out_f32 && (a.ldo_f32 % 4 || !al(a.out_f32, 16))) return false;
   if (a.out_t && (a.ldo_t % 4 || !al(a.out_t, 4 * sizeof(E)) || (Opnd<T>::NP == 2 && a.out_t_lo_off % 4))) return false;
   if (a.resid && (a.ldr % 4 || !al(a.resid, 16))) return false;
@@ -871,9 +902,21 @@
   }
   return true;
 }
+static int gemm_pitch_of(const fdm_gemm_args& a) {
+  const int pitch = FDM_TILE_PITCH(a.tile);
+  if (pitch <= 0 || pitch >= 64 || (a.tile & (FDM_TILE_GENERAL | FDM_TILE_NO_PITCH))) return 0;
+  if (a.ksplit > 1 || a.batch2 >= 1 || a.out_kp || a.out_vp || a.stat_out || a.ln_stat_in || a.K >= (1 << 24)) return 0;
+  return pitch;
+}
 template <typename T, int BM, int BN, int WM, int WN, int NST, int KCH, int LW>
 static hipError_t gemm_glds_launch_lw(const fdm_gemm_args& a, hipStream_t s) {
   const bool no_lean = (a.tile & FDM_TILE_GENERAL) != 0;
+  if constexpr (BM == 64 && (BN == 64 || BN == 128) && NST >= 3) {
+    if (gemm_pitch_of(a) && gemm_all_tiles_lean<T, BM, BN>(a, true)) {
+      if (gemm_act_is_heavy(a.act)) return gemm_glds_launch_h<T, BM, BN, WM, WN, NST, KCH, true, false, GEMM_LEAN | GEMM_PITCH, LW>(a, s);
+      return gemm_glds_launch_h<T, BM, BN, WM, WN, NST, KCH, false, false, GEMM_LEAN | GEMM_PITCH, LW>(a, s);
+    }
+  }
   if (a.ksplit > 1) {
     if constexpr (BN == 64 && (BM == 64 || BM == 32)) {
       if (!gemm_all_tiles_lean<T, BM, BN>(a)) return hipErrorInvalidValue;
@@ -945,6 +988,27 @@
 static bool gemm_one_round_64x128(const fdm_gemm_args& a) {
   const long long t = (long long)((a.M + 63) / 64) * ((a.N + 127) / 128) * (a.batch > 0 ? a.batch : 1);
   return gemm_one_round(t) && a.N >= 2048 && a.N % 128 == 0;
+}
+
+static bool gemm_pitch_env_on() {
+  static bool v = [] { const char* e = getenv("FDM_ROW_PITCH"); return e && atoi(e) != 0; }();
+  return v;
+}
+static int gemm_propose_pitch(const fdm_gemm_args& a, int bn, int min_pitch) {
+  if (a.ksplit > 1 || a.batch2 >= 1 || a.out_kp || a.out_vp || a.stat_out || a.ln_stat_in || a.resid_row_mod) return 0;
+  if (a.M < 64 || a.N % bn || a.K >= (1 << 24)) return 0;
+  const long long cols = (long long)(a.N / bn) * (a.batch > 0 ? a.batch : 1);
+  const long long nb = (a.M + 63) / 64;
+  if (cols > 256 || nb * cols >= 256) return 0;
+  const long long nb2 = 256 / cols;
+  if (nb2 <= nb) return 0;
+  const int pitch = (int)((a.M + nb2 - 1) / nb2);
+  return (pitch >= min_pitch && pitch < 64) ? pitch : 0;
+}
+static int gemm_heuristic_pitch(const fdm_gemm_args& a, int tile_id, int elem_bytes) {
+  if (elem_bytes != 2 || !gemm_pitch_env_on() || (a.tile & FDM_TILE_NO_PITCH)) return 0;
+  if (tile_id != FDM_TILE_64x64 && tile_id != FDM_TILE_64x128) return 0;
+  return gemm_propose_pitch(a, tile_id == FDM_TILE_64x64 ? 64 : 128, 48);
 }
 
 static int gemm_heuristic_tile(const fdm_gemm_args& a, int elem_bytes, bool split) {
@@ -1020,13 +1084,23 @@
   if constexpr (LM == 0) {
     if (a.sched.mode == 3) return gemm_sched_fuse_launch<T, GEMM_LM>(a, s);
   }
+  const bool pitched = gemm_pitch_of(a) != 0;
   if constexpr (!std::is_same<T, float>::value) {
     if (!(a.tile & FDM_TILE_LOCKSTEP) && !gemm_lockstep_env())
-      return a.ln_stat_in ? gemm_glds_launch_h<T, 64, 64, 2, 4, 4, 8, false, true, GEMM_LEAN | GEMM_FOLD | LM, 4>(a, s)
+      return pitched      ? gemm_glds_launch_h<T, 64, 64, 2, 4, 4, 8, false, true, GEMM_LEAN | GEMM_PITCH | LM, 4>(a, s)
+           : a.ln_stat_in ? gemm_glds_launch_h<T, 64, 64, 2, 4, 4, 8, false, true, GEMM_LEAN | GEMM_FOLD | LM, 4>(a, s)
                           : gemm_glds_launch_h<T, 64, 64, 2, 4, 4, 8, false, true, GEMM_LEAN | LM, 4>(a, s);
   }
+  if (pitched) return gemm_glds_launch_h<T, 64, 64, 2, 4, 4, 8, false, true, GEMM_LEAN | GEMM_PITCH | LM>(a, s);
   return a.ln_stat_in ? gemm_glds_launch_h<T, 64, 64, 2, 4, 4, 8, false, true, GEMM_LEAN | GEMM_FOLD | LM>(a, s)
                       : gemm_glds_launch_h<T, 64, 64, 2, 4, 4, 8, false, true, GEMM_LEAN | LM>(a, s);
+}
+
+static fdm_gemm_args gemm_with_pitch(const fdm_gemm_args& a, int resolved_id, int elem_bytes) {
+  fdm_gemm_args b = a;
+  const int pitch = (a.tile & FDM_TILE_ID_MASK) ? FDM_TILE_PITCH(a.tile) : gemm_heuristic_pitch(a, resolved_id, elem_bytes);
+  b.tile = (a.tile & ~(FDM_TILE_PITCH_MASK << FDM_TILE_PITCH_SHIFT)) | (pitch << FDM_TILE_PITCH_SHIFT);
+  return b;
 }
 
 static int gemm_ksplit_heuristic_tile(const fdm_gemm_args& a) { return a.M <= 256 ? FDM_TILE_32x64_S3 : FDM_TILE_64x64; }
@@ -1040,8 +1114,10 @@
 }
 
 template <typename T>
-static hipError_t gemm_dispatch(const fdm_gemm_args& a, hipStream_t s) {
-  if (a.sched_fuse) {
+static hipError_t gemm_dispatch(const fdm_gemm_args& a_in, hipStream_t s) {
+  constexpr int EB = (int)sizeof(typename Opnd<T>::E);
+  if (a_in.sched_fuse) {
+    const fdm_gemm_args a = gemm_with_pitch(a_in, FDM_TILE_64x64, EB);
     const int tile_id = a.tile & FDM_TILE_ID_MASK;
     const bool pp = tile_id == FDM_TILE_256x128_PP || (tile_id == 0 && gemm_tile_override() == 0 && gemm_sched_fuse_heuristic_pp(a, (int)sizeof(typename Opnd<T>::E)));
     if (pp && !a.ln_stat_in && a.N % 128 == 0)
@@ -1049,10 +1125,12 @@
                                : gemm_pp_launch_h<T, 256, 128, 4, 2, 3, false, true, GEMM_LEAN>(a, s);
     return gemm_sched_fuse_launch<T>(a, s);
   }
-  const int tile_id = a.tile & FDM_TILE_ID_MASK;
-  if (a.ksplit > 1) return gemm_dispatch_ksplit<T>(a, tile_id, s);
-  const int want = tile_id > 0 ? tile_id : (a.batch2 >= 1 ? 0 : gemm_tile_override());
-  switch (want > 0 ? want : gemm_heuristic_tile(a, (int)sizeof(typename Opnd<T>::E), false)) {
+  const int tile_id = a_in.tile & FDM_TILE_ID_MASK;
+  if (a_in.ksplit > 1) return gemm_dispatch_ksplit<T>(a_in, tile_id, s);
+  const int want = tile_id > 0 ? tile_id : (a_in.batch2 >= 1 ? 0 : gemm_tile_override());
+  const int resolved = want > 0 ? want : gemm_heuristic_tile(a_in, EB, false);
+  const fdm_gemm_args a = gemm_with_pitch(a_in, resolved, EB);
+  switch (resolved) {
     case FDM_TILE_128x64_S3:
     case FDM_TILE_128x64: {
       const long long wgs = (long long)((a.M + 127) / 128) * ((a.N + 63) / 64) * (a.batch > 0 ? a.batch : 1) * (a.batch2 > 0 ? a.batch2 : 1);
@@ -1071,13 +1149,15 @@
 }
 
 template <typename T>
-static hipError_t gemm_dispatch_split(const fdm_gemm_args& a, hipStream_t s) {
-  if (a.sched_fuse)
-    return gemm_sched_fuse_launch<T>(a, s);
-  const int tile_id = a.tile & FDM_TILE_ID_MASK;
-  if (a.ksplit > 1) return gemm_dispatch_ksplit<T>(a, tile_id, s);
-  const int want = tile_id > 0 ? tile_id : (a.batch2 >= 1 ? 0 : gemm_tile_override());
-  switch (want > 0 ? want : gemm_heuristic_tile(a, 2, true)) {
+static hipError_t gemm_dispatch_split(const fdm_gemm_args& a_in, hipStream_t s) {
+  if (a_in.sched_fuse)
+    return gemm_sched_fuse_launch<T>(gemm_with_pitch(a_in, FDM_TILE_64x64, 2), s);
+  const int tile_id = a_in.tile & FDM_TILE_ID_MASK;
+  if (a_in.ksplit > 1) return gemm_dispatch_ksplit<T>(a_in, tile_id, s);
+  const int want = tile_id > 0 ? tile_id : (a_in.batch2 >= 1 ? 0 : gemm_tile_override());
+  const int resolved = want > 0 ? want : gemm_heuristic_tile(a_in, 2, true);
+  const fdm_gemm_args a = gemm_with_pitch(a_in, resolved, 2);
+  switch (resolved) {
     case FDM_TILE_64x64_S2: return gemm_glds_launch_t<T, 64, 64, 2, 4, 2, 4>(a, s);
     case FDM_TILE_32x64_S3: return gemm_glds_launch_t<T, 32, 64, 2, 2, 3, 2>(a, s);
     case FDM_TILE_128x64:
diff --git a/face-diffusion-model_amd/csrc/gemm_bf16.hip b/face-diffusion-model_amd/csrc/gemm_bf16.hip
--- a/face-diffusion-model_amd/csrc/gemm_bf16.hip
+++ b/face-diffusion-model_amd/csrc/gemm_bf16.hip
@@ -2,14 +2,22 @@
 #include "kernels.hpp"
 namespace fdm { hipError_t gemm_launch_bf16(const fdm_gemm_args& a, hipStream_t s) { return gemm_dispatch<bf16>(a, s); } }
 namespace fdm {
-int gemm_heuristic_tile_of(const fdm_gemm_args& a) {
+int gemm_heuristic_tile_of(const fdm_gemm_args& a_in) {
+  fdm_gemm_args a = a_in;
+  a.tile = 0;
+  const int eb = a.dtype == FDM_F32 ? 4 : 2;
+  auto with_pitch = [&](int id) { return FDM_TILE_WITH_PITCH(id, gemm_pitch_of(gemm_with_pitch(a, id, eb))); };
   if (a.ksplit > 1) return gemm_ksplit_heuristic_tile(a);
   if (a.sched_fuse) {
-    const bool pp = a.dtype != FDM_F16X3 && gemm_tile_override() == 0 && !a.ln_stat_in && a.N % 128 == 0 && gemm_sched_fuse_heuristic_pp(a, a.dtype == FDM_F32 ? 4 : 2);
-    return pp ? FDM_TILE_256x128_PP : FDM_TILE_64x64;
+    const bool pp = a.dtype != FDM_F16X3 && gemm_tile_override() == 0 && !a.ln_stat_in && a.N % 128 == 0 && gemm_sched_fuse_heuristic_pp(a, eb);
+    return pp ? FDM_TILE_256x128_PP : with_pitch(FDM_TILE_64x64);
   }
   const int want = gemm_tile_override();
-  if (want > 0) return want;
-  return gemm_heuristic_tile(a, a.dtype == FDM_F32 ? 4 : 2, a.dtype == FDM_F16X3);
+  return with_pitch(want > 0 ? want : gemm_heuristic_tile(a, eb, a.dtype == FDM_F16X3));
+}
+int gemm_candidate_pitch(const fdm_gemm_args& a, int tile_id) {
+  if (tile_id != FDM_TILE_64x64 && tile_id != FDM_TILE_64x128) return 0;
+  if (a.sched_fuse && tile_id != FDM_TILE_64x64) return 0;
+  return gemm_propose_pitch(a, tile_id == FDM_TILE_64x64 ? 64 : 128, 32);
 }
 }
diff --git a/face-diffusion-model_amd/csrc/kernels.hpp b/face-diffusion-model_amd/csrc/kernels.hpp
--- a/face-diffusion-model_amd/csrc/kernels.hpp
+++ b/face-diffusion-model_amd/csrc/kernels.hpp
@@ -9,6 +9,7 @@
 hipError_t gemm_launch_f16x3(const fdm_gemm_args& a, hipStream_t s);
 hipError_t gemm_launch_f16(const fdm_gemm_args& a, hipStream_t s);
 int gemm_heuristic_tile_of(const fdm_gemm_args& a);
+int gemm_candidate_pitch(const fdm_gemm_args& a, int tile_id);
 hipError_t attn_launch_f32(const fdm_attn_args& a, hipStream_t s);
 hipError_t attn_launch_bf16(const fdm_attn_args& a, hipStream_t s);
 hipError_t attn_launch_f16x3(const fdm_attn_args& a, hipStream_t s);
diff --git a/face-diffusion-model_amd/csrc/plan.hip b/face-diffusion-model_amd/csrc/plan.hip
--- a/face-diffusion-model_amd/csrc/plan.hip
+++ b/face-diffusion-model_amd/csrc/plan.hip
@@ -79,10 +79,16 @@
 void set_ksplit(fdm_gemm_args& g, int S, long long plane) { if (S > 1) { g.ksplit = S; g.ksplit_stride = plane; } }
 void set_ksplit(fdm_ln_args& ln, int S, long long plane) { if (S > 1) { ln.x_planes = S; ln.x_plane_stride = plane; } }
 
+}
+int fdm::plan_tile(const fdm_plan* P, int tile) {
+  if (P->row_pitch > 0 && !(tile & FDM_TILE_ID_MASK)) tile = FDM_TILE_WITH_PITCH(FDM_TILE_64x64, P->row_pitch);
+  return tile | (P->lockstep ? FDM_TILE_LOCKSTEP : 0) | (P->row_pitch < 0 ? FDM_TILE_NO_PITCH : 0);
+}
+namespace {
 int plan_gemm(fdm_plan* P, const char* label, fdm_gemm_args a, void* stream) {
   if (P->tune_rec) (*P->tune_rec)[label].push_back(a);
   auto it = P->tiles.find(label);
-  a.tile = (it == P->tiles.end() ? 0 : it->second) | (P->lockstep ? FDM_TILE_LOCKSTEP : 0);
+  a.tile = plan_tile(P, it == P->tiles.end() ? 0 : it->second);
   return fdm_op_gemm(&a, stream);
 }
 
@@ -406,7 +412,7 @@
   std::string s;
   for (auto& kv : P->tiles)
     if (kv.second) s += kv.first + "=" + std::to_string(kv.second) + ",";
-  s += "ks" + std::to_string(P->ksplit_out) + std::to_string(P->ksplit_ffn2) + (P->lockstep ? "L" : "");
+  s += "ks" + std::to_string(P->ksplit_out) + std::to_string(P->ksplit_ffn2) + (P->lockstep ? "L" : "") + (P->row_pitch ? "p" + std::to_string(P->row_pitch) : "");
   return s;
 }
 
@@ -1431,6 +1437,7 @@
   else if (k == "rows") *out = P->R;
   else if (k == "ksplit.out") *out = P->ksplit_out;
   else if (k == "ksplit.ffn2") *out = P->ksplit_ffn2;
+  else if (k == "row_pitch") *out = P->row_pitch;
   else if (k == "tuned") *out = P->tile_cache.count(shape_key(P)) ? 1 : 0;
   else if (k == "needs_tune") *out = needs_tune(P, shape_key(P)) ? 1 : 0;
   else if (k == "tune_failed") *out = P->tune_failed;
@@ -1481,12 +1488,18 @@
     return FDM_OK;
   }
   if (k == "lockstep") { P->lockstep = value != 0; P->tile_cache.clear(); P->tiles.clear(); return drop_programs(P, nullptr); }
+  if (k == "row_pitch") {
+    if (value < -1 || value > 63) return fail(FDM_ERR_ARG, "plan_set: row_pitch = %lld outside -1..63", value);
+    if (P->row_pitch == (int)value) return FDM_OK;
+    P->row_pitch = (int)value; P->tile_cache.clear(); P->tiles.clear();
+    return drop_programs(P, nullptr);
+  }
   if (k == "untune") {
     P->tile_cache.clear(); P->steps_seen.clear(); P->tiles.clear(); P->tune_failed_shapes.clear();
     return drop_programs(P, nullptr);
   }
   if (k.rfind("tile.", 0) == 0) {
-    if (value < 0 || value > FDM_TILE_MAX) return fail(FDM_ERR_ARG, "plan_set: unknown tile %lld", value);
+    if (!tile_value_ok(value)) return fail(FDM_ERR_ARG, "plan_set: unknown tile %lld", value);
     P->tiles[k.substr(5)] = (int)value;
     P->tile_cache[shape_key(P)] = P->tiles;
     return drop_programs(P, nullptr);
diff --git a/face-diffusion-model_amd/csrc/plan.hpp b/face-diffusion-model_amd/csrc/plan.hpp
--- a/face-diffusion-model_amd/csrc/plan.hpp
+++ b/face-diffusion-model_amd/csrc/plan.hpp
@@ -45,6 +45,7 @@
   std::map<std::string, long long> steps_seen;
   std::map<std::string, std::vector<fdm_gemm_args>>* tune_rec = nullptr;
   int tune_enabled = 1;
+  int row_pitch = 0;
   int tune_failed = 0;
   std::set<std::string> tune_failed_shapes;
   int want_fuse_ln3 = 0;
@@ -94,6 +95,12 @@
 int record_chain(fdm_plan* P, const fdm_sched_args* sched, void* stream);
 bool needs_tune(fdm_plan* P, const std::string& key);
 int tune_tiles(fdm_plan* P, int force, void* stream);
+int plan_tile(const fdm_plan* P, int tile);
+inline bool tile_value_ok(long long v) {
+  if (v < 0 || (v & ~(long long)(FDM_TILE_ID_MASK | (FDM_TILE_PITCH_MASK << FDM_TILE_PITCH_SHIFT)))) return false;
+  const int id = (int)v & FDM_TILE_ID_MASK, pitch = FDM_TILE_PITCH((int)v);
+  return id <= FDM_TILE_MAX && pitch < 64 && (pitch == 0 || id == FDM_TILE_64x64 || id == FDM_TILE_64x128);
+}
 void tune_soft(fdm_plan* P, void* stream);
 void select_tiles(fdm_plan* P);
 }
diff --git a/face-diffusion-model_amd/csrc/tune.hip b/face-diffusion-model_amd/csrc/tune.hip
--- a/face-diffusion-model_amd/csrc/tune.hip
+++ b/face-diffusion-model_amd/csrc/tune.hip
@@ -45,7 +45,7 @@
 std::string store_key(const fdm_plan* P) {
   const fdm_model_desc& m = P->m;
   char b[160];
-  snprintf(b, sizeof(b), "v%d|dt%d|%d,%d,%d,%d,%d,%d,%d,%d|%s", fdm_version(), P->dtype, m.d, m.n_head, m.n_layers, m.ffn, m.G, m.c, m.audio_in, m.pair,
+  snprintf(b, sizeof(b), "v%d.p1.%d|dt%d|%d,%d,%d,%d,%d,%d,%d,%d|%s", fdm_version(), P->row_pitch, P->dtype, m.d, m.n_head, m.n_layers, m.ffn, m.G, m.c, m.audio_in, m.pair,
            shape_key(P).c_str());
   return b;
 }
@@ -69,7 +69,7 @@
   if (it == lines.end()) return false;
   tiles.clear();
   for (auto& kv : parse_tiles(it->second)) {
-    if (kv.second < 0 || kv.second > FDM_TILE_MAX) return false;
+    if (!tile_value_ok(kv.second)) return false;
     if (kv.second) tiles[kv.first] = kv.second;
   }
   return true;
@@ -121,7 +121,7 @@
       fdm_prog* prog = nullptr;
       FCK(fdm_prog_create(&prog));
       int rc = fdm_prog_begin(prog);
-      for (size_t i = 0; rc == FDM_OK && i < inst.size(); ++i) { fdm_gemm_args a = inst[i]; a.tile = tile | (P->lockstep ? FDM_TILE_LOCKSTEP : 0); a.incr_counter = nullptr; a.incr_table = nullptr; rc = fdm_op_gemm(&a, stream); }
+      for (size_t i = 0; rc == FDM_OK && i < inst.size(); ++i) { fdm_gemm_args a = inst[i]; a.tile = plan_tile(P, tile); a.incr_counter = nullptr; a.incr_table = nullptr; rc = fdm_op_gemm(&a, stream); }
       (void)fdm_prog_end(prog);
       float ms = 0.f;
       if (rc == FDM_OK) rc = time_prog(prog, 2, 5, s, &ms);
@@ -132,10 +132,11 @@
     }
     return FDM_OK;
   };
-  std::vector<int> cands = {FDM_TILE_64x64, FDM_TILE_64x64_S2, FDM_TILE_32x64_S3, FDM_TILE_128x64, FDM_TILE_128x128, FDM_TILE_80x128, FDM_TILE_64x128};
-  if (!split && P->R >= 1024) cands.push_back(FDM_TILE_256x128_PP);
+  std::vector<int> base_cands = {FDM_TILE_64x64, FDM_TILE_64x64_S2, FDM_TILE_32x64_S3, FDM_TILE_128x64, FDM_TILE_128x128, FDM_TILE_80x128, FDM_TILE_64x128};
+  if (!split && P->R >= 1024) base_cands.push_back(FDM_TILE_256x128_PP);
   struct Geo { int bm, bn, nst; };
   auto geo = [&](int tile) -> Geo {
+    if (FDM_TILE_PITCH(tile)) return {FDM_TILE_PITCH(tile), (tile & FDM_TILE_ID_MASK) == FDM_TILE_64x128 ? 128 : 64, (split && (tile & FDM_TILE_ID_MASK) == FDM_TILE_64x128) ? 3 : 4};
     switch (tile) {
       case FDM_TILE_64x64_S2: return {64, 64, 2};
       case FDM_TILE_32x64_S3: return {32, 64, 3};
@@ -163,16 +164,21 @@
     FCK(timed(inst, 0, &base));
     std::vector<std::pair<float, int>> cand = {{base * 0.97f, 0}};
     double best_model = 1e30;
+    std::vector<int> cands = base_cands;
+    if (P->row_pitch >= 0)
+      for (int id : {FDM_TILE_64x64, FDM_TILE_64x128})
+        if (const int pitch = gemm_candidate_pitch(kv.second[0], id)) cands.push_back(FDM_TILE_WITH_PITCH(id, pitch));
     for (int tile : cands) best_model = std::min(best_model, modelled_us(kv.second[0], tile));
     auto launched = [&](int tile) {
       if (!split) return tile;
       return tile == FDM_TILE_256x128_PP ? FDM_TILE_128x128 : tile;
     };
-    const int heur = launched(fdm_gemm_heuristic_tile(&kv.second[0]));
+    const int heur = launched(gemm_heuristic_tile_of(kv.second[0]));
     for (int tile : cands) {
       if (launched(tile) == heur) continue;
-      if (kv.second[0].ksplit > 1 && tile != FDM_TILE_64x64 && tile != FDM_TILE_64x64_S2 && tile != FDM_TILE_32x64_S3) continue;
-      if (kv.second[0].sched_fuse && tile != FDM_TILE_256x128_PP && tile != FDM_TILE_64x64) continue;
+      const int id = tile & FDM_TILE_ID_MASK;
+      if (kv.second[0].ksplit > 1 && id != FDM_TILE_64x64 && id != FDM_TILE_64x64_S2 && id != FDM_TILE_32x64_S3) continue;
+      if (kv.second[0].sched_fuse && id != FDM_TILE_256x128_PP && id != FDM_TILE_64x64) continue;
       if (modelled_us(kv.second[0], tile) > 1.35 * best_model) continue;
       float t = 0.f;
       FCK(timed(inst, tile, &t));
diff --git a/face-diffusion-model_amd/fdm_amd/_lib.py b/face-diffusion-model_amd/fdm_amd/_lib.py
--- a/face-diffusion-model_amd/fdm_amd/_lib.py
+++ b/face-diffusion-model_amd/fdm_amd/_lib.py
@@ -43,6 +43,15 @@
 
 TILE_AUTO, TILE_64x64, TILE_128x64, TILE_128x128, TILE_64x64_S2, TILE_32x64_S3, TILE_256x128_PP, TILE_80x128, TILE_64x128 = 0, 1, 2, 3, 8, 9, 10, 11, 12
 TILE_96x128, TILE_256x128, TILE_64x64_S3, TILE_128x64_S3 = 4, 5, 6, 7
+TILE_NO_PITCH = 0x400
+
+
+def tile_with_pitch(tile, pitch):
+    return tile | (pitch << 16)
+
+
+def tile_pitch(tile):
+    return (tile >> 16) & 0x7f
 
 
 class ModelDesc(C.Structure):
diff --git a/include/fdm_hip.h b/include/fdm_hip.h
--- a/include/fdm_hip.h
+++ b/include/fdm_hip.h
@@ -113,6 +113,11 @@
 #define FDM_TILE_GENERAL 0x100
 #define FDM_TILE_LOCKSTEP 0x200
 #define FDM_TILE_ID_MASK 0xff
+#define FDM_TILE_PITCH_SHIFT 0x10
+#define FDM_TILE_PITCH_MASK 0x7f
+#define FDM_TILE_PITCH(tile) (((tile) >> FDM_TILE_PITCH_SHIFT) & FDM_TILE_PITCH_MASK)
+#define FDM_TILE_WITH_PITCH(id, pitch) ((id) | ((pitch) << FDM_TILE_PITCH_SHIFT))
+#define FDM_TILE_NO_PITCH 0x400
 int fdm_op_gemm(const fdm_gemm_args* a, void* stream);
 int fdm_gemm_heuristic_tile(const fdm_gemm_args* a);
 
```

After: 1935 frames/s. 0.962x the previous value.
